# thunlp/OpenMatch

Measured on AMD Instinct MI355X. Metric: passages/sec encode (bert-base DPR bi-encoder, 128 tok -> 768-d) [+ queries/sec exact top-1000 over 8.8M x 768 in `search`], higher is better.
Workload: dtype f16; 1 GPU; bert-base DPR bi-encoder encode+search, MS MARCO 8.8M x 128-tok -> 768-d (BASELINE configs[1]); seq_len=128, global_batch=1024, index_rows=8841823, queries=6980, topk=1000, weights=random-init BertConfig() seed 0, parallelism=shard1

## Files before the change

include/openmatch_hip.h:

```cpp
#ifndef OPENMATCH_HIP_H
#define OPENMATCH_HIP_H

#include <stddef.h>
#include <stdint.h>

#ifdef __cplusplus
extern "C" {
#endif

#define OM_ABI_VERSION 6

#define OM_F32 0
#define OM_BF16 1
#define OM_F16 2

#define OM_ACT_NONE 0
#define OM_ACT_GELU_ERF 1
#define OM_ACT_RELU 2
#define OM_ACT_GELU_TANH 3
#define OM_ACT_SILU 5
#define OM_ACT_MUL_RESID 0x100
#define OM_ACT_PRE_GRAD 0x200

#define OM_ARCH_BERT 0
#define OM_ARCH_T5 1
#define OM_ARCH_MODERNBERT 2

#define OM_ARCH_CAUSAL 3

#define OM_ARCH_NOMICBERT 4

#define OM_POOL_NONE 0
#define OM_POOL_FIRST 1
#define OM_POOL_MEAN 2
#define OM_POOL_LAST 3

#define OM_SEARCH_F32 0
#define OM_SEARCH_F16_RESCORE 1

const char* om_last_error(void);
int om_abi_version(void);

int om_device_count(void);

#define OM_TIMING_GEMM_BF16 0
#define OM_TIMING_GEMM_F32 1
#define OM_TIMING_SCAN 2
void om_debug_gemm_trace(unsigned long long* buf);
void om_debug_gemm_gen(int gen);
#define OM_GEMM_FAMILY_V1 1
#define OM_GEMM_FAMILY_V2 2
#define OM_GEMM_FAMILY_V6 6
#define OM_GEMM_FAMILY_G7 7
#define OM_GEMM_FAMILY_G7_ONE_TILE 70
#define OM_GEMM_FAMILY_G7C16 71
#define OM_GEMM_FAMILY_G7R16 72
#define OM_GEMM_FAMILY_SKINNY 9
int om_debug_gemm_last(void);
int om_debug_gemm_plan(int in_dtype, const void* A, int64_t lda, const void* B, int64_t ldb, int out_dtype, void* C, int64_t ldc,
                       int64_t M, int64_t N, int64_t K, const float* bias, const void* resid, int64_t ldr, int act);
typedef struct OmDebugGemmEpilogue {
  const float* bias; const void* resid; int64_t ldr; int act;
  void* pre_act; int64_t ldp; float drop_p; uint64_t seed; const int* drop_rows;
  const float* ln_stats; const float* ln_colsum; const float* rln_stats; const float* rln_g; const float* rln_b; float* stats_out;
  const void* resid_lo; void* out_lo;
  const float* resid32; float* out32;
  const float* a_ln32; const float* a_ln_g; const float* a_ln_b; float* a_ln_stats_out; const float* rln32; const float* rln32_stats;
  int lo8; float ln_inv_h, ln_eps; int ln_rms; int reverse;
  const int* rows_dev;
} OmDebugGemmEpilogue;
int om_debug_gemm_ex(int in_dtype, const void* A, int64_t lda, const void* B, int64_t ldb, int out_dtype, void* C, int64_t ldc,
                     int64_t M, int64_t N, int64_t K, const OmDebugGemmEpilogue* ep, void* stream);
int om_debug_gemm_plan_ex(int in_dtype, const void* A, int64_t lda, const void* B, int64_t ldb, int out_dtype, void* C, int64_t ldc,
                          int64_t M, int64_t N, int64_t K, const OmDebugGemmEpilogue* ep);
int om_debug_gemm_splitk(int in_dtype, const void* A, int64_t lda, const void* B, int64_t ldb, float* C, int64_t ldc, int64_t M,
                         int64_t N, int64_t K, void* stream);
#define OM_OPT_ENCODER_FUSED_LN 0
#define OM_OPT_ENCODER_DEBUG 1
#define OM_OPT_ATTENTION_FAST 2
#define OM_OPT_SCAN_GEN7 3
#define OM_OPT_SCAN_GROWTH 4
#define OM_OPT_WGRAD_DEBUG 5
#define OM_OPT_GEMM_GROUP_M 6
#define OM_OPT_SCAN_QGROUP 7
#define OM_OPT_TRAIN_WGRAD_STREAM 8
#define OM_OPT_ATTENTION_DEBUG 9
#define OM_OPT_ENCODER_PINGPONG 10
#define OM_OPT_ENCODER_TWO_PLANE 11
#define OM_OPT_GEMM_VARIANT 12
#define OM_OPT_SEARCH_DEBUG 13
#define OM_OPT_TRAIN_WGRAD_BATCH 14
#define OM_OPT_GEMM_MAX_GRID 15
#define OM_OPT_GEMM_CONT 16
#define OM_OPT_TRAIN_TAPE_GRAD 17
#define OM_OPT_TRAIN_RES32 18
#define OM_OPT_GEMM_SKINNY_M 19
#define OM_OPT_GEMM_SKINNY_CFG 20
#define OM_OPT_FEW_ROWS_LN_FUSE 21
#define OM_OPT_ENCODER_SKIP_PAD 22
#define OM_OPT_COUNT 23
int om_debug_option(int opt, int value);
int om_debug_option_value(int opt);
int om_debug_attention(const void* qkv, void* ctx, const int64_t* mask, int64_t B, int L, int H, int heads, void* stream);
int om_debug_attention_ex(int dtype, const void* qkv, void* ctx, const int64_t* mask, const float* pos_bias, int64_t B, int L, int H,
                          int heads, float scale, float drop_p, uint64_t seed, void* stream, int reverse, const int* kmax,
                          const int* cu, int w);
int om_debug_rope(int dtype, void* qkv, int64_t M, int L, int H, float theta, void* stream);
int om_debug_rope_rows(int dtype, void* qkv, int64_t rows, int L, int H, float theta, const int* row_map, void* stream);
int om_debug_swiglu_rows(int dtype, const void* in, void* out, int64_t M, int F, void* stream);
int om_debug_embed(int dtype, const int64_t* ids, const int64_t* type_ids, const float* word, const float* pos, const float* type,
                   const float* g, const float* b, void* out, int64_t M, int L, int H, int vocab, int type_vocab, float eps, void* stream);
int om_debug_attention_causal(int dtype, const void* qkv, void* ctx, const int64_t* mask, int64_t B, int L, int n_heads, int n_kv_heads,
                              float scale, void* stream);
int om_debug_rope_gqa(int dtype, void* qkv, int64_t M, int L, int n_heads, int n_kv_heads, const float* inv_freq, float scaling, void* stream);
int om_debug_attention_causal_packed(int dtype, const void* qkv, void* ctx, const int64_t* mask, const int* cu, int64_t B, int L, int n_heads,
                                     int n_kv_heads, float scale, void* stream);
int om_debug_rope_gqa_rows(int dtype, void* qkv, int64_t rows, int L, int n_heads, int n_kv_heads, const float* inv_freq, float scaling,
                           const int* row_map, void* stream);
int om_debug_attention_causal_hd(int dtype, const void* qkv, void* ctx, const int64_t* mask, int64_t B, int L, int n_heads, int n_kv_heads,
                                 int head_dim, float scale, void* stream);
int om_debug_attention_causal_hd_packed(int dtype, const void* qkv, void* ctx, const int64_t* mask, const int* cu, int64_t B, int L,
                                        int n_heads, int n_kv_heads, int head_dim, float scale, void* stream);
int om_debug_qknorm_rope(int dtype, void* qkv, int64_t M, int L, int n_heads, int n_kv_heads, int head_dim, const float* q_norm_g,
                         const float* k_norm_g, float eps, const float* inv_freq, float scaling, void* stream);
int om_debug_qknorm_rope_rows(int dtype, void* qkv, int64_t rows, int L, int n_heads, int n_kv_heads, int head_dim, const float* q_norm_g,
                              const float* k_norm_g, float eps, const float* inv_freq, float scaling, const int* row_map, void* stream);
int om_debug_attention_gqa_d256(int dtype, const void* qkv, void* ctx, const int64_t* mask, int64_t B, int L, int n_heads, int n_kv_heads,
                                float scale, int w, void* stream);
int om_debug_qknorm_rope_d256(int dtype, void* qkv, int64_t M, int L, int n_heads, int n_kv_heads, const float* q_norm_g, const float* k_norm_g,
                              float eps, const float* inv_freq, float scaling, void* stream);
int om_debug_attention_gqa_d256_packed(int dtype, const void* qkv, void* ctx, const int64_t* mask, const int* cu, int64_t B, int L, int n_heads,
                                       int n_kv_heads, float scale, int w, void* stream);
int om_debug_qknorm_rope_d256_rows(int dtype, void* qkv, int64_t rows, int L, int n_heads, int n_kv_heads, const float* q_norm_g,
                                   const float* k_norm_g, float eps, const float* inv_freq, float scaling, const int* row_map, void* stream);
int om_debug_rmsnorm_add(int dtype, const void* h, int64_t ldh, float* x, int64_t ldx, const float* g, int64_t M, int H, float eps, void* stream);
int om_debug_mask_extent(const int64_t* mask, int64_t B, int L, int* kmax, void* stream);
int om_debug_pack_rows(const int* kmax, int64_t B, int L, int64_t rows, int* cu, int* cls_rows, int* row_map, void* stream);
#define OM_ATTN_FAMILY_GENERIC 1
#define OM_ATTN_FAMILY_FWD16 2
#define OM_ATTN_FAMILY_FWD16_KMAX4 3
#define OM_ATTN_FAMILY_FWD16C 4
#define OM_ATTN_FAMILY_LONG 5
#define OM_ATTN_FAMILY_D32 6
#define OM_ATTN_FAMILY_BAND16 7
#define OM_ATTN_FAMILY_BAND32 8
int om_debug_attention_last(void);
int om_debug_attention_plan(int dtype, int64_t B, int L, int H, int heads, int has_bias, float drop_p, int has_kmax, int has_cu, int w);
#define OM_ATTN_BWD_FAMILY_BWD16 1
#define OM_ATTN_BWD_FAMILY_GENERIC 2
#define OM_ATTN_BWD_FAMILY_LONG 3
#define OM_ATTN_BWD_FAMILY_D32 4
int om_debug_attention_bwd_last(void);
int om_debug_attention_bwd_plan(int dtype, int64_t B, int L, int H, int heads, int has_bias, int has_drel, int has_cu, int packed);
int om_debug_attention_bwd_ex(int dtype, const void* qkv, const void* ctx, const void* dctx, void* dqkv, const int64_t* mask,
                              const float* pos_bias, float* drel, float* stats, int64_t B, int L, int H, int heads, float scale,
                              float drop_p, uint64_t seed, const int* cu, int packed, void* stream);
size_t om_debug_attention_bwd_stats_bytes(int64_t B, int heads);
#define OM_ENC_PATH_BERT_FUSED 1
#define OM_ENC_PATH_BERT_PENDING_LN 2
#define OM_ENC_PATH_BERT_FEW32 3
#define OM_ENC_PATH_BERT_PLAIN 4
#define OM_ENC_PATH_MODERNBERT 5
#define OM_ENC_PATH_T5_FUSED 6
#define OM_ENC_PATH_T5_PLAIN 7
struct OmEncoderConfig;
int om_debug_encoder_plan(const struct OmEncoderConfig* cfg, int gated_ffn, int has_rel_bias, int64_t B, int64_t L, int64_t packed_rows,
                          int want_hidden);
int om_debug_encoder_skip_pad(const struct OmEncoderConfig* cfg, int gated_ffn, int has_rel_bias, int64_t B, int64_t L, int want_hidden);
int om_debug_attn_drop_keep(uint64_t seed, int64_t b, int h, int heads, int Lm, int q, int key, float p);
int om_debug_wave_sum_check(const float* in, float* out_shuffle, float* out_dpp, int64_t groups, void* stream);
#define OM_ROW_FWD_GENERIC 1
#define OM_ROW_FWD_X8 2
#define OM_ROW_LN_BWD 3
int om_debug_row_kernel_last(void);
int om_debug_layernorm(int dtype, const void* x, int64_t ldx, void* y, int64_t ldy, const float* g, const float* b, int64_t M, int H,
                       float eps, int rms, const void* x_lo, int lo8, void* stream);
int om_debug_layernorm_f32out(int dtype, const void* x, int64_t ldx, float* y, int64_t ldy, const float* g, const float* b, int64_t M,
                              int H, float eps, int rms, const void* x_lo, const int* rows, int lo8, void* stream);
int om_debug_layernorm_from_f32(int dtype, const float* x, int64_t ldx, void* y, int64_t ldy, const float* g, const float* b, int64_t M,
                                int H, float eps, int rms, void* stream);
int om_debug_layernorm_dual(int dtype, const float* x, int64_t ldx, void* y, float* y32, int64_t ldy, const float* g, const float* b,
                            int64_t M, int H, float eps, void* stream);
int om_debug_norm_bwd(int dtype, const void* dy, const void* x, const float* g, void* dx, float* dg, float* db, int64_t M, int H,
                      float eps, int rms, const void* add, void* stream);
int om_debug_ln_bwd_drop(int dtype, const void* dy, const void* x, const float* g, void* dx, void* dx_drop, float drop_p,
                         uint64_t drop_seed, float* dg, float* db, int64_t M, int H, float eps, const float* dy32, const float* x32,
                         float* partial, int* partial_blocks , const int* drop_rows, void* stream);
typedef struct OmLnSite { const float* partial; float* dg; float* db; int blocks; } OmLnSite;
int om_debug_ln_param_reduce(const OmLnSite* sites , int n, int H, void* stream);
int om_debug_embed_bwd(int dtype, const void* dy, const int64_t* ids, const int64_t* type_ids, const float* word, const float* pos,
                       const float* type, const float* g, float* dword, float* dpos, float* dtype_, float* dg, float* db, int64_t M,
                       int L, int H, int vocab, int type_vocab, float eps, const int* cu, void* stream);
int om_debug_pool(int dtype, const void* x, const int64_t* mask, float* out, int64_t B, int L, int H, int mode, const int* cu,
                  void* stream);
int om_debug_pool_bwd(int dtype, const float* dp, const int64_t* mask, void* dh, int64_t B, int L, int H, int mode, const int* cu,
                      void* stream);
int om_debug_l2norm(const float* x, float* y, int64_t M, int D, void* stream);
int om_debug_l2norm_bwd(const float* x, const float* dy, float* dx, int64_t M, int D, void* stream);
int om_debug_colsum(int dtype, const void* x, int64_t ld, int64_t M, int N, float* out, void* stream);
int om_debug_dropout(int dtype, const void* x, void* y, int64_t n, float p, uint64_t seed, const int* rows, int H, void* stream);
int om_debug_ln_fold(int dtype, const void* W, const float* gamma, const float* beta, const float* b, void* Wf, float* colsum,
                     float* bf, int N, int K, void* stream);
int om_debug_ln_stats_reduce(const float* slots, int nslots, int64_t M, float* out, void* stream);
int om_kernel_timing_enable(int enable);
int om_kernel_timing_read(int kernel_class, double* total_ms, int64_t* launches, double* flops);

int om_gemm_nt(int in_dtype, const void* A, int64_t lda, const void* B, int64_t ldb,
               int out_dtype, void* C, int64_t ldc, int64_t M, int64_t N, int64_t K,
               const float* bias, const void* resid, int64_t ldr, int act, void* stream);

int om_gemm_tn_acc(int in_dtype, const void* A, int64_t lda, const void* B, int64_t ldb,
                   float* C, int64_t ldc, float* bias, int64_t M, int64_t N, int64_t K, void* stream);

typedef struct OmTnProblem {
  const void* A; const void* B; float* C; float* bias;
  int64_t lda, ldb, ldc, N, K;
} OmTnProblem;
int om_gemm_tn_acc_batch(int in_dtype, const OmTnProblem* problems, int n, int64_t M, void* stream);

typedef struct OmLayerWeights {
  const void* qkv_w;
  const float* qkv_b;
  const void* o_w;
  const float* o_b;
  const float* ln1_g;
  const float* ln1_b;
  const void* ffn1_w;
  const float* ffn1_b;
  const void* ffn1g_w;
  const void* ffn2_w;
  const float* ffn2_b;
  const float* ln2_g;
  const float* ln2_b;
} OmLayerWeights;

typedef struct OmEncoderConfig {
  int arch;
  int dtype;
  int hidden;
  int n_layers;
  int n_heads;
  int head_dim;
  int ffn;
  int vocab;
  int max_pos;
  int type_vocab;
  int act;
  float ln_eps;
  int rel_buckets;
  int rel_max_dist;
  int pooling;
  int head_in;
  int head_out;
  int normalize;
  float rope_theta_global;
  float rope_theta_local;
  int half_window;
  uint64_t sliding_layers;
} OmEncoderConfig;

typedef struct OmEncoderWeights {
  const float* word_emb;
  const float* pos_emb;
  const float* type_emb;
  const float* emb_ln_g;
  const float* emb_ln_b;
  const OmLayerWeights* layers_host;
  const float* final_ln_g;
  const float* rel_bias;
  const float* head_w;
  const void* folded;
  const float* final_ln_b;
} OmEncoderWeights;

size_t om_encoder_fold_bytes(const OmEncoderConfig* cfg);
int om_encoder_fold_weights(const OmEncoderConfig* cfg, const OmEncoderWeights* w, void* folded, size_t bytes, void* stream);

size_t om_encoder_workspace_bytes(const OmEncoderConfig* cfg, int64_t B, int64_t L);

int om_t5_relative_bucket(int relative_position, int num_buckets, int max_distance);

int om_encoder_forward(const OmEncoderConfig* cfg, const OmEncoderWeights* w,
                       const int64_t* input_ids, const int64_t* attention_mask,
                       const int64_t* token_type_ids, int64_t B, int64_t L,
                       void* out_hidden, float* out_reps, void* workspace,
                       size_t workspace_bytes, void* stream);

int om_encoder_packed_supported(const OmEncoderConfig* cfg, int gated_ffn, int64_t B, int64_t L, int64_t packed_rows);
size_t om_encoder_workspace_bytes_packed(const OmEncoderConfig* cfg, int64_t B, int64_t L, int64_t packed_rows);
int om_encoder_forward_packed(const OmEncoderConfig* cfg, const OmEncoderWeights* w,
                              const int64_t* input_ids, const int64_t* attention_mask,
                              const int64_t* token_type_ids, int64_t B, int64_t L, int64_t packed_rows,
                              float* out_reps, void* workspace, size_t workspace_bytes, void* stream);

typedef struct OmCausalConfig {
  OmEncoderConfig base;
  int n_kv_heads;
  float rope_attention_scaling;
  float inv_freq[32];
} OmCausalConfig;
size_t om_causal_encoder_workspace_bytes(const OmCausalConfig* cfg, int64_t B, int64_t L);
int om_causal_encoder_forward(const OmCausalConfig* cfg, const OmEncoderWeights* w, const int64_t* input_ids,
                              const int64_t* attention_mask, int64_t B, int64_t L, void* out_hidden, float* out_reps,
                              void* workspace, size_t workspace_bytes, void* stream);
int om_causal_encoder_packed_supported(const OmCausalConfig* cfg, int64_t B, int64_t L, int64_t packed_rows);
size_t om_causal_encoder_workspace_bytes_packed(const OmCausalConfig* cfg, int64_t B, int64_t L, int64_t packed_rows);
int om_causal_encoder_forward_packed(const OmCausalConfig* cfg, const OmEncoderWeights* w, const int64_t* input_ids,
                                     const int64_t* attention_mask, int64_t B, int64_t L, int64_t packed_rows, float* out_reps,
                                     void* workspace, size_t workspace_bytes, void* stream);

typedef struct OmCausalConfig2 {
  OmCausalConfig base;
  int qk_norm;
  int reserved;
  float inv_freq[64];
} OmCausalConfig2;
typedef struct OmCausalQkNorm {
  const float* q_norm_g;
  const float* k_norm_g;
} OmCausalQkNorm;
size_t om_causal2_encoder_workspace_bytes(const OmCausalConfig2* cfg, int64_t B, int64_t L);
// ... 204 lines not shown
```

openmatch_amd/csrc/abi.cpp:

```cpp
#include "common.h"

static thread_local std::string g_last_error;
void om_set_error(const std::string& msg) { g_last_error = msg; }

extern "C" const char* om_last_error(void) { return g_last_error.c_str(); }
extern "C" int om_abi_version(void) { return OM_ABI_VERSION; }
extern "C" int om_device_count(void) {
  int n = 0;
  hipError_t e = hipGetDeviceCount(&n);
  if (e != hipSuccess) {
    om_set_error(std::string("hipGetDeviceCount: ") + hipGetErrorString(e));
    return -1;
  }
  return n;
}

#include <mutex>
#include <vector>
namespace {
struct Span { hipEvent_t a, b; };
struct ClassStat { std::vector<Span> spans; double flops = 0; size_t used = 0; };
bool g_timing = false;
ClassStat g_stat[3];
std::mutex g_mu;
}
bool om_timing_on() { return g_timing; }
void om_timing_begin(int c, hipStream_t s) {
  std::lock_guard<std::mutex> lk(g_mu);
  ClassStat& st = g_stat[c];
  if (st.used == st.spans.size()) {
    Span sp;
    (void)hipEventCreate(&sp.a);
    (void)hipEventCreate(&sp.b);
    st.spans.push_back(sp);
  }
  (void)hipEventRecord(st.spans[st.used].a, s);
}
void om_timing_end(int c, hipStream_t s, double flops) {
  std::lock_guard<std::mutex> lk(g_mu);
  ClassStat& st = g_stat[c];
  (void)hipEventRecord(st.spans[st.used].b, s);
  st.used++;
  st.flops += flops;
}
extern "C" int om_kernel_timing_enable(int enable) { g_timing = enable != 0; return 0; }
extern "C" int om_kernel_timing_read(int c, double* total_ms, int64_t* launches, double* flops) {
  if (c < 0 || c > 2) { om_set_error("om_kernel_timing_read: bad class"); return 1; }
  std::lock_guard<std::mutex> lk(g_mu);
  ClassStat& st = g_stat[c];
  double ms = 0;
  for (size_t i = 0; i < st.used; ++i) {
    hipError_t e = hipEventSynchronize(st.spans[i].b);
    float t = 0;
    if (e == hipSuccess) e = hipEventElapsedTime(&t, st.spans[i].a, st.spans[i].b);
    if (e != hipSuccess) { om_set_error(std::string("om_kernel_timing_read: ") + hipGetErrorString(e)); return 1; }
    ms += t;
  }
  if (total_ms) *total_ms = ms;
  if (launches) *launches = (int64_t)st.used;
  if (flops) *flops = st.flops;
  st.used = 0; st.flops = 0;
  return 0;
}

#include <atomic>
#include <map>
#include <tuple>
namespace {
std::atomic<int> g_opt[OM_OPT_COUNT];
std::atomic<bool> g_opt_init{false};
std::mutex g_opt_mu;
void opt_init() {
  std::lock_guard<std::mutex> lk(g_opt_mu);
  if (g_opt_init.load()) return;
  const char* e = getenv("OM_ENCODER_FUSED_LN");
  g_opt[OM_OPT_ENCODER_FUSED_LN] = e ? atoi(e) : 1;
  g_opt[OM_OPT_ENCODER_DEBUG] = getenv("OM_ENCODER_DEBUG") ? 1 : 0;
  e = getenv("OM_ATTENTION_FAST");
  g_opt[OM_OPT_ATTENTION_FAST] = e ? atoi(e) : 1;
  e = getenv("OM_SCAN_GEN7");
  g_opt[OM_OPT_SCAN_GEN7] = e ? atoi(e) : 1;
  e = getenv("OM_SCAN_GROWTH");
  g_opt[OM_OPT_SCAN_GROWTH] = e ? atoi(e) : 60;
  g_opt[OM_OPT_WGRAD_DEBUG] = 0;
  g_opt[OM_OPT_ATTENTION_DEBUG] = 0;
  e = getenv("OM_ENCODER_PINGPONG");
  g_opt[OM_OPT_ENCODER_PINGPONG] = e ? atoi(e) : 1;
  e = getenv("OM_TRAIN_WGRAD_STREAM");
  g_opt[OM_OPT_TRAIN_WGRAD_STREAM] = e ? atoi(e) : 1;
  e = getenv("OM_SCAN_QGROUP");
  g_opt[OM_OPT_SCAN_QGROUP] = e ? atoi(e) : 8;
  e = getenv("OM_GEMM_GROUP_M");
  g_opt[OM_OPT_GEMM_GROUP_M] = e ? atoi(e) : 8;
  e = getenv("OM_ENCODER_TWO_PLANE");
  g_opt[OM_OPT_ENCODER_TWO_PLANE] = e ? atoi(e) : 3;
  e = getenv("OM_GEMM_VARIANT");
  g_opt[OM_OPT_GEMM_VARIANT] = e ? atoi(e) : 0;
  e = getenv("OM_SEARCH_DEBUG");
  g_opt[OM_OPT_SEARCH_DEBUG] = e ? (atoi(e) ? atoi(e) : 1) : 0;
  e = getenv("OM_TRAIN_WGRAD_BATCH");
  g_opt[OM_OPT_TRAIN_WGRAD_BATCH] = e ? atoi(e) : 4;
  e = getenv("OM_GEMM_MAX_GRID");
  g_opt[OM_OPT_GEMM_MAX_GRID] = e ? atoi(e) : 0;
  e = getenv("OM_TRAIN_TAPE_GRAD");
  g_opt[OM_OPT_TRAIN_TAPE_GRAD] = e ? atoi(e) : 1;
  e = getenv("OM_TRAIN_RES32");
  g_opt[OM_OPT_TRAIN_RES32] = e ? atoi(e) : 1;
  e = getenv("OM_GEMM_CONT");
  g_opt[OM_OPT_GEMM_CONT] = e ? atoi(e) : 495;
  e = getenv("OM_GEMM_SKINNY_M");
  g_opt[OM_OPT_GEMM_SKINNY_M] = e ? atoi(e) : 1024;
  e = getenv("OM_FEW_ROWS_LN_FUSE");
  g_opt[OM_OPT_FEW_ROWS_LN_FUSE] = e ? atoi(e) : 64;
  e = getenv("OM_ENCODER_SKIP_PAD");
  g_opt[OM_OPT_ENCODER_SKIP_PAD] = e ? atoi(e) : 1;
  g_opt_init.store(true);
}
}
bool om_option_is_set(int opt) {
  if (opt == OM_OPT_SCAN_GROWTH) return getenv("OM_SCAN_GROWTH") != nullptr;
  return false;
}
int om_option(int opt) {
  if (!g_opt_init.load(std::memory_order_acquire)) opt_init();
  return g_opt[opt].load(std::memory_order_relaxed);
}
extern "C" int om_debug_option(int opt, int value) {
  if (opt < 0 || opt >= OM_OPT_COUNT) { om_set_error("om_debug_option: unknown option"); return 1; }
  if (!g_opt_init.load(std::memory_order_acquire)) opt_init();
  g_opt[opt].store(value);
  return 0;
}
extern "C" int om_debug_option_value(int opt) {
  if (opt < 0 || opt >= OM_OPT_COUNT) { om_set_error("om_debug_option_value: unknown option"); return -1; }
  return om_option(opt);
}

int om_t5_lut_device(int L, int buckets, int max_dist, const int** out) {
  static std::mutex mu;
  static std::map<std::tuple<int, int, int, int>, int*> cache;
  int dev = 0;
  OM_HIP(hipGetDevice(&dev));
  std::lock_guard<std::mutex> lk(mu);
  auto key = std::make_tuple(dev, L, buckets, max_dist);
  auto it = cache.find(key);
  if (it == cache.end()) {
    std::vector<int> lut(2 * L);
    for (int rel = -(L - 1); rel <= L - 1; ++rel) lut[rel + (L - 1)] = om_t5_relative_bucket(rel, buckets, max_dist);
    int* d = nullptr;
    OM_HIP(hipMalloc(&d, (size_t)(2 * L) * sizeof(int)));
    OM_HIP(hipMemcpy(d, lut.data(), (size_t)(2 * L - 1) * sizeof(int), hipMemcpyHostToDevice));
    it = cache.emplace(key, d).first;
  }
  *out = it->second;
  return 0;
}
```

openmatch_amd/csrc/attention.hip:

```cpp
#include <type_traits>

#include "attn_chunked.h"
#include "attn_plan.h"

static thread_local int g_attn_last = 0;
extern "C" int om_debug_attention_last(void) { return g_attn_last; }

template <typename T, int KT>
__global__ __launch_bounds__(64 * KT) void attention_kernel(
    const T* __restrict__ qkv, T* __restrict__ ctx, const int64_t* __restrict__ mask,
    const float* __restrict__ pos_bias, int L, int H, int heads, float scale, float drop_p,
    uint64_t seed) {
  typedef AttnGeom<T> G;
  typedef typename MmaOps<T>::frag_t frag_t;
  constexpr int LP = KT * 32 + 4;
  extern __shared__ __attribute__((aligned(16))) char smem[];
  char* sK = smem;
  T* sVt = (T*)(smem + KT * 32 * G::ROWB);
  float* sM = (float*)(smem + KT * 32 * G::ROWB + 64 * LP * (int)sizeof(T));

  const int h = blockIdx.x % heads;
  const int64_t b = blockIdx.x / heads;
  const int tid = threadIdx.x, nthr = blockDim.x;
  const int64_t ld = 3 * (int64_t)H;
// ... 262 lines not shown
    }
  char* const out = (char*)(ctx + (row0 + q0) * (int64_t)H + h * 64);
#pragma unroll
  for (int it = 0; it < 4; ++it) {
    const int row = it * 8 + (lane >> 3), c = lane & 7;
    const uint4 v = *(const uint4*)(so + row * 128 + ((c ^ (row & 7)) << 4));
    if (!(DBG & 4) || v.x == 0x12345u) { if (q0 + row < L) *(uint4*)(out + (int64_t)row * H * 2 + c * 16) = v; }
  }
}

template <typename T, int KT, bool BIAS, bool DROP, int DBG = 0>
__global__ __launch_bounds__(64 * KT, KT <= 4 ? ((BIAS || DROP) ? 3 : 4) : 2) void attention_fwd16_kernel(
    const T* __restrict__ qkv, T* __restrict__ ctx, const int64_t* __restrict__ mask,
    const float* __restrict__ pos_bias, int L, int H, int heads, float scale, float drop_p, uint64_t seed, int rev,
    const int* __restrict__ kmax, const int* __restrict__ cu) {
#define OM_ATTN_BODY(V) attention_fwd16_body<T, KT, BIAS, DROP, DBG, V>(qkv, ctx, mask, pos_bias, Lb, H, heads, scale, drop_p, seed, rev, row0, L)
  const int64_t b = rev ? (int64_t)(gridDim.x / heads) - 1 - blockIdx.x / heads : blockIdx.x / heads;
  int64_t row0 = b * L;
  int Lb = L;
  if (cu) {
    const int c0 = __builtin_amdgcn_readfirstlane(cu[b]), c1 = __builtin_amdgcn_readfirstlane(cu[b + 1]);
    row0 = c0; Lb = c1 - c0;
    if (Lb <= 0) return;
  }
  if (KT == 4 && !BIAS && !DROP && (kmax || cu)) {
    const int kt = ((cu ? Lb : __builtin_amdgcn_readfirstlane(kmax[b])) + 31) >> 5;
    if (kt <= 1) { OM_ATTN_BODY(1); return; }
    if (kt == 2) { OM_ATTN_BODY(2); return; }
    if (kt == 3) { OM_ATTN_BODY(3); return; }
  }
  OM_ATTN_BODY(KT);
#undef OM_ATTN_BODY
}

template <typename T, int KT, bool BIAS, bool DROP>
static int launch_attn16(const void* qkv, void* ctx, const int64_t* mask, const float* pos_bias, int64_t B, int L, int H,
                         int heads, float scale, float drop_p, uint64_t seed, hipStream_t s, int rev, const int* kmax, const int* cu) {
  const int lds = 2 * KT * 32 * 128 + KT * 32 * 4;
  if (attn_lds_once<attention_fwd16_kernel<T, KT, BIAS, DROP>>(lds)) return 1;
#ifdef OM_PROBE_KERNELS
  const int dbg = (sizeof(T) == 2 && std::is_same<T, bf16_t>::value && KT == 4 && !BIAS && !DROP) ? om_option(OM_OPT_ATTENTION_DEBUG) : 0;
#else
  const int dbg = 0;
#endif
  if (dbg) {
#ifdef OM_PROBE_KERNELS
#define OM_ATTN_DBG(D)                                                                                                        \
  case D:                                                                                                                     \
    hipLaunchKernelGGL((attention_fwd16_kernel<bf16_t, 4, false, false, D>), dim3((unsigned)(heads * B)), dim3(256), lds, s,          \
                       (const bf16_t*)qkv, (bf16_t*)ctx, mask, pos_bias, L, H, heads, scale, drop_p, seed, rev, kmax, cu);    \
    break;
    switch (dbg) { OM_ATTN_DBG(1) OM_ATTN_DBG(2) OM_ATTN_DBG(3) OM_ATTN_DBG(4) OM_ATTN_DBG(5) OM_ATTN_DBG(6) OM_ATTN_DBG(7) default: break; }
#undef OM_ATTN_DBG
#endif
    OM_LAUNCH_CHECK();
    return 0;
  }
  hipLaunchKernelGGL((attention_fwd16_kernel<T, KT, BIAS, DROP>), dim3((unsigned)(heads * B)), dim3(64 * KT), lds, s, (const T*)qkv,
                     (T*)ctx, mask, pos_bias, L, H, heads, scale, drop_p, seed, rev, kmax, cu);
  OM_LAUNCH_CHECK();
  return 0;
}
template <typename T, bool BIAS, bool DROP>
__global__ __launch_bounds__(256, 2) void attention_fwd16c_kernel(
    const T* __restrict__ qkv, T* __restrict__ ctx, const int64_t* __restrict__ mask,
    const float* __restrict__ pos_bias, int Lm, int H, int heads, float scale, float drop_p, uint64_t seed, const int* __restrict__ cu) {
  const int h = blockIdx.x % heads;
  const int64_t b = blockIdx.x / heads;
  int64_t row0 = b * Lm;
  int L = Lm;
  if (cu) {
    const int c0 = __builtin_amdgcn_readfirstlane(cu[b]), c1 = __builtin_amdgcn_readfirstlane(cu[b + 1]);
    row0 = c0; L = c1 - c0;
  }
  const int qb = blockIdx.y * 128;
  if (qb >= L) return;
  attn_chunked16<T, AttnFull, BIAS, DROP>(attn_rows_fused(qkv, ctx, row0, H, h), AttnFull{}, mask + b * Lm, L, L, qb, scale, AttnFullArgs{pos_bias, drop_p, seed, b, h, heads, Lm});
}

template <typename T, bool BIAS, bool DROP>
static int launch_attn16c(const void* qkv, void* ctx, const int64_t* mask, const float* pos_bias, int64_t B, int L, int H,
                           int heads, float scale, float drop_p, uint64_t seed, hipStream_t s, const int* cu) {
  const int lds = 2 * 128 * 128 + 128 * 4;
  hipLaunchKernelGGL((attention_fwd16c_kernel<T, BIAS, DROP>), dim3((unsigned)(heads * B), (unsigned)((L + 127) / 128)), dim3(256), lds, s,
                     (const T*)qkv, (T*)ctx, mask, pos_bias, L, H, heads, scale, drop_p, seed, cu);
  OM_LAUNCH_CHECK();
  return 0;
}
template <typename T>
__global__ __launch_bounds__(256) void attention_long_kernel(
    const T* __restrict__ qkv, T* __restrict__ ctx, const int64_t* __restrict__ mask,
    const float* __restrict__ pos_bias, int Lm, int H, int heads, float scale, float drop_p, uint64_t seed, const int* __restrict__ cu) {
  const int h = blockIdx.x % heads;
  const int64_t b = blockIdx.x / heads;
  const int qb = blockIdx.y * 128;
  int64_t row0 = b * Lm;
  int L = Lm;
  if (cu) { row0 = cu[b]; L = cu[b + 1] - cu[b]; }
  if (qb >= L) return;
  attn_chunked_qreg<T, AttnFull>(attn_rows_fused(qkv, ctx, row0, H, h), AttnFull{}, mask + b * Lm, L, L, qb, scale, AttnFullArgs{pos_bias, drop_p, seed, b, h, heads, Lm});
}

template <typename T>
static int launch_attn_long(const void* qkv, void* ctx, const int64_t* mask, const float* pos_bias, int64_t B, int L, int H,
                            int heads, float scale, float drop_p, uint64_t seed, hipStream_t s, const int* cu) {
  const int lds = 128 * AttnGeom<T>::ROWB + 64 * 132 * (int)sizeof(T) + 128 * 4 + 128 * 4;
  if (attn_lds_once<attention_long_kernel<T>>(lds)) return 1;
  hipLaunchKernelGGL((attention_long_kernel<T>), dim3((unsigned)(heads * B), (unsigned)((L + 127) / 128)), dim3(256), lds, s,
                     (const T*)qkv, (T*)ctx, mask, pos_bias, L, H, heads, scale, drop_p, seed, cu);
  OM_LAUNCH_CHECK();
  return 0;
}

template <typename T, int KT>
static int launch_attn(const void* qkv, void* ctx, const int64_t* mask, const float* pos_bias,
                       int64_t B, int L, int H, int heads, float scale, float drop_p, uint64_t seed,
                       hipStream_t s) {
  constexpr int LP = KT * 32 + 4;
  const int lds = KT * 32 * AttnGeom<T>::ROWB + 64 * LP * (int)sizeof(T) + KT * 32 * 4;
  if (attn_lds_once<attention_kernel<T, KT>>(lds)) return 1;
  const int waves = (L + 31) / 32;
  hipLaunchKernelGGL((attention_kernel<T, KT>), dim3((unsigned)(heads * B)),
                     dim3(64 * waves), lds, s, (const T*)qkv, (T*)ctx, mask, pos_bias, L, H, heads,
                     scale, drop_p, seed);
  OM_LAUNCH_CHECK();
  return 0;
}

__global__ void mask_extent_kernel(const int64_t* __restrict__ mask, int64_t B, int L, int* __restrict__ kmax) {
  const int64_t b = (int64_t)blockIdx.x * (blockDim.x >> 6) + (threadIdx.x >> 6);
  if (b >= B) return;
  const int lane = threadIdx.x & 63;
  int last = 0;
  for (int k = lane; k < L; k += 64) if (mask[b * L + k] != 0) last = k + 1;
#pragma unroll
  for (int o = 32; o > 0; o >>= 1) last = max(last, __shfl_xor(last, o, 64));
  if (lane == 0) kmax[b] = last ? last : L;
}
__global__ __launch_bounds__(1024) void pack_rows_kernel(const int* __restrict__ kmax, int64_t B, int L, int64_t rows, int* __restrict__ cu,
                                                          int* __restrict__ cls_rows, int* __restrict__ row_map) {
  __shared__ int part[1024];
  const int tid = threadIdx.x;
  const int64_t per = (B + 1023) / 1024, lo = tid * per, hi = lo + per < B ? lo + per : B;
  int sum = 0;
  for (int64_t i = lo; i < hi; ++i) sum += kmax[i];
  part[tid] = sum;
  __syncthreads();
  for (int off = 1; off < 1024; off <<= 1) {
    const int v = tid >= off ? part[tid - off] : 0;
    __syncthreads();
    part[tid] += v;
    __syncthreads();
  }
  int run = part[tid] - sum;
  const int cap = (int)rows;
  for (int64_t i = lo; i < hi; ++i) {
    cu[i] = run < cap ? run : cap;
    cls_rows[i] = run < cap ? run : cap - 1;
    const int n = kmax[i];
    for (int k = 0; k < n; ++k) if (run + k < cap) row_map[run + k] = (int)(i * L + k);
    run += n;
  }
  const int total = part[1023];
  if (tid == 1023) { cu[B] = total < cap ? total : cap; cu[B + 1] = total; }
  for (int64_t t = total + tid; t < rows; t += 1024) row_map[t] = -1;
}
int omk_pack_rows(const int* kmax, int64_t B, int L, int64_t rows, int* cu, int* cls_rows, int* row_map, hipStream_t s) {
  if (B <= 0) return 0;
  if (rows > 0x7fffffff || B * (int64_t)L > 0x7fffffff) OM_FAIL("packed rows: token counts below 2^31");
  hipLaunchKernelGGL(pack_rows_kernel, dim3(1), dim3(1024), 0, s, kmax, B, L, rows, cu, cls_rows, row_map);
  OM_LAUNCH_CHECK();
  return 0;
}

int omk_mask_extent(const int64_t* mask, int64_t B, int L, int* kmax, hipStream_t s) {
  if (B <= 0) return 0;
  hipLaunchKernelGGL(mask_extent_kernel, dim3((unsigned)((B + 3) / 4)), dim3(256), 0, s, mask, B, L, kmax);
  OM_LAUNCH_CHECK();
  return 0;
}

int omk_attention(int dtype, const void* qkv, void* ctx, const int64_t* mask, const float* pos_bias, int64_t B, int L, int H, int heads,
                  float scale, float drop_p, uint64_t seed, hipStream_t s, int reverse, const int* kmax, const int* cu, int w) {
  g_attn_last = 0;
  const AttnPlan p = attn_plan_fwd(dtype, B, L, H, heads, pos_bias != nullptr, drop_p, kmax != nullptr, cu != nullptr, w, attn_switches());
  if (p.error) OM_FAIL(p.error);
  g_attn_last = p.family | (p.kt << 8);
  switch (p.family) {
    case 0: return 0;
    case OM_ATTN_FAMILY_D32: return omk_attention_d32(p, dtype, qkv, ctx, mask, pos_bias, B, L, H, heads, scale, drop_p, seed, s, reverse, kmax, cu);
    case OM_ATTN_FAMILY_BAND16: case OM_ATTN_FAMILY_BAND32: return omk_attention_band(dtype, qkv, ctx, mask, B, L, H, heads, scale, w, kmax, s);
    case OM_ATTN_FAMILY_FWD16: case OM_ATTN_FAMILY_FWD16_KMAX4:
      return attn_with_type16(dtype, [&](auto t) {
        return attn_with_kt<1, 2, 4, 6, 8>(p.kt, [&](auto kt) {
          return attn_with_flags(p.bias, p.drop, [&](auto bias, auto drop) {
            return launch_attn16<decltype(t), kt(), bias(), drop()>(qkv, ctx, mask, pos_bias, B, L, H, heads, scale, drop_p, seed, s, reverse, kmax, cu);
          });
        });
      });
    case OM_ATTN_FAMILY_FWD16C:
      return attn_with_type16(dtype, [&](auto t) {
        return attn_with_flags(p.bias, p.drop, [&](auto bias, auto drop) {
          return launch_attn16c<decltype(t), bias(), drop()>(qkv, ctx, mask, pos_bias, B, L, H, heads, scale, drop_p, seed, s, cu);
        });
      });
    case OM_ATTN_FAMILY_LONG:
      return attn_with_type(dtype, [&](auto t) { return launch_attn_long<decltype(t)>(qkv, ctx, mask, pos_bias, B, L, H, heads, scale, drop_p, seed, s, cu); });
    default:
      if (dtype == OM_BF16)
        return attn_with_kt<1, 2, 4, 6, 8>(p.kt, [&](auto kt) { return launch_attn<bf16_t, kt()>(qkv, ctx, mask, pos_bias, B, L, H, heads, scale, drop_p, seed, s); });
      return attn_with_kt<1, 2, 4, 6, 8>(p.kt, [&](auto kt) { return launch_attn<float, kt()>(qkv, ctx, mask, pos_bias, B, L, H, heads, scale, drop_p, seed, s); });
  }
}

extern "C" int om_debug_attention_plan(int dtype, int64_t B, int L, int H, int heads, int has_bias, float drop_p, int has_kmax, int has_cu, int w) {
  const AttnPlan p = attn_plan_fwd(dtype, B, L, H, heads, has_bias != 0, drop_p, has_kmax != 0, has_cu != 0, w, attn_switches());
  if (p.error) { om_set_error(std::string(__func__) + ": " + p.error); return -1; }
  return p.family | (p.kt << 8);
}

extern "C" int om_debug_attention_ex(int dtype, const void* qkv, void* ctx, const int64_t* mask, const float* pos_bias, int64_t B, int L, int H,
                                     int heads, float scale, float drop_p, uint64_t seed, void* stream, int reverse, const int* kmax,
                                     const int* cu, int w) {
  g_attn_last = 0;
  if (!qkv || !ctx || !mask) OM_FAIL("null argument");
  if (dtype != OM_F32 && dtype != OM_BF16 && dtype != OM_F16) OM_FAIL("attention: dtype must be OM_F32, OM_BF16 or OM_F16");
  if (w > 0 && (pos_bias || drop_p > 0.f || cu || reverse)) OM_FAIL("banded attention: no position bias, dropout, packed rows or reverse walk");
  return omk_attention(dtype, qkv, ctx, mask, pos_bias, B, L, H, heads, scale, drop_p, seed, (hipStream_t)stream, reverse, kmax, cu, w);
}
extern "C" int om_debug_attention(const void* qkv, void* ctx, const int64_t* mask, int64_t B, int L, int H, int heads, void* stream) {
  return om_debug_attention_ex(OM_BF16, qkv, ctx, mask, nullptr, B, L, H, heads, 0.125f, 0.f, 0, stream, 0, nullptr, nullptr, 0);
}
extern "C" int om_debug_rope(int dtype, void* qkv, int64_t M, int L, int H, float theta, void* stream) {
  if (!qkv) OM_FAIL("null argument");
  if (dtype != OM_F32 && dtype != OM_BF16 && dtype != OM_F16) OM_FAIL("rotary positions: dtype must be OM_F32, OM_BF16 or OM_F16");
  return omk_rope(dtype, qkv, M, L, H, theta, (hipStream_t)stream);
}
extern "C" int om_debug_rope_rows(int dtype, void* qkv, int64_t rows, int L, int H, float theta, const int* row_map, void* stream) {
  if (!qkv || !row_map) OM_FAIL("null argument");
  if (dtype != OM_F32 && dtype != OM_BF16 && dtype != OM_F16) OM_FAIL("rotary positions: dtype must be OM_F32, OM_BF16 or OM_F16");
  return omk_rope(dtype, qkv, rows, L, H, theta, (hipStream_t)stream, row_map);
}
extern "C" int om_debug_mask_extent(const int64_t* mask, int64_t B, int L, int* kmax, void* stream) {
  if (!mask || !kmax) OM_FAIL("null argument");
  if (L < 1) OM_FAIL("mask extent: L must be at least 1");
  return omk_mask_extent(mask, B, L, kmax, (hipStream_t)stream);
}
extern "C" int om_debug_pack_rows(const int* kmax, int64_t B, int L, int64_t rows, int* cu, int* cls_rows, int* row_map, void* stream) {
  if (!kmax || !cu || !cls_rows || !row_map) OM_FAIL("null argument");
  if (rows < 1) OM_FAIL("packed rows: rows must be at least 1");
  return omk_pack_rows(kmax, B, L, rows, cu, cls_rows, row_map, (hipStream_t)stream);
}
extern "C" int om_debug_attn_drop_keep(uint64_t seed, int64_t b, int h, int heads, int Lm, int q, int key, float p) {
  return attn_drop_keep1(seed, b, h, heads, Lm, q, key, AttnDrop(p).thresh) ? 1 : 0;
}
```

openmatch_amd/csrc/elementwise.hip:

```cpp
#include "common.h"
#include "kernels.h"
#include "ln_row.h"
#include <type_traits>

#define ROWS_PER_BLOCK 4
#define MAX_VEC_LIMIT 8

template <typename TOut, int MAX_VEC>
__device__ inline void norm_and_store(float (&x)[MAX_VEC][4], int nvec, int lane, int H,
                                      const float* __restrict__ g, const float* __restrict__ b,
                                      float eps, int rms, TOut* __restrict__ out, float* __restrict__ out32 = nullptr) {
  float mean, rstd;
  ln_row_stats<MAX_VEC>(x, nvec, lane, H, eps, rms, mean, rstd);
#pragma unroll
  for (int j = 0; j < MAX_VEC; ++j) {
    const int c = (lane + 64 * j) * 4;
    if (j < nvec && c < H) {
      float gv[4], y[4];
      Vec4<float>::load(g + c, gv);
      if (b) {
        float bv[4];
        Vec4<float>::load(b + c, bv);
#pragma unroll
        for (int e = 0; e < 4; ++e) y[e] = ln_affine(x[j][e], mean, rstd, gv[e], bv[e]);
// ... 178 lines not shown
  float v[MAX_VEC][4];
  if (bert) {
    int64_t tt = type_ids ? type_ids[row] : 0;
    tt = tt < 0 ? 0 : (tt >= type_vocab ? type_vocab - 1 : tt);
    const int t = (int)(row % L);
#pragma unroll
    for (int j = 0; j < MAX_VEC; ++j) {
      const int c = (lane + 64 * j) * 4;
      if (j < nvec && c < H) {
        float w[4], ty[4], p[4];
        Vec4<float>::load(word + id * H + c, w);
        if (type && pos) {
          Vec4<float>::load(type + tt * H + c, ty);
          Vec4<float>::load(pos + (int64_t)t * H + c, p);
#pragma unroll
          for (int e = 0; e < 4; ++e) v[j][e] = (w[e] + ty[e]) + p[e];
        } else if (type) {
          Vec4<float>::load(type + tt * H + c, ty);
#pragma unroll
          for (int e = 0; e < 4; ++e) v[j][e] = w[e] + ty[e];
        } else if (pos) {
          Vec4<float>::load(pos + (int64_t)t * H + c, p);
#pragma unroll
          for (int e = 0; e < 4; ++e) v[j][e] = w[e] + p[e];
        } else {
#pragma unroll
          for (int e = 0; e < 4; ++e) v[j][e] = w[e];
        }
      }
    }
    norm_and_store<TOut, MAX_VEC>(v, nvec, lane, H, g, b, eps, 0, out + orow * H, out32 ? out32 + orow * H : nullptr);
  } else {
#pragma unroll
    for (int j = 0; j < MAX_VEC; ++j) {
      const int c = (lane + 64 * j) * 4;
      if (j < nvec && c < H) {
        Vec4<float>::load(word + id * H + c, v[j]);
        Vec4<TOut>::store(out + orow * H + c, v[j]);
      }
    }
  }
}

template <typename T>
__global__ void pool_kernel(const T* __restrict__ x, const int64_t* __restrict__ mask,
                            float* __restrict__ out, int L, int H, int mode, const int* __restrict__ cu) {
  const int64_t b = blockIdx.x;
  const T* xb = x + (cu ? (int64_t)cu[b] : b * (int64_t)L) * H;
  const int Lb = cu ? cu[b + 1] - cu[b] : L;
  for (int c = threadIdx.x * 4; c < H; c += blockDim.x * 4) {
    float acc[4] = {0.f, 0.f, 0.f, 0.f};
    if (mode == OM_POOL_FIRST) {
      Vec4<T>::load(xb + c, acc);
    } else {
      float cnt = 0.f;
      for (int t = 0; t < Lb; ++t) {
        const float m = (float)mask[b * L + t];
        float v[4];
        Vec4<T>::load(xb + (int64_t)t * H + c, v);
#pragma unroll
        for (int e = 0; e < 4; ++e) acc[e] += v[e] * m;
        cnt += m;
      }
      cnt = fmaxf(cnt, 1e-9f);
#pragma unroll
      for (int e = 0; e < 4; ++e) acc[e] = acc[e] / cnt;
    }
    Vec4<float>::store(out + b * H + c, acc);
  }
}

__global__ __launch_bounds__(64 * ROWS_PER_BLOCK) void l2norm_kernel(const float* __restrict__ x,
                                                                     float* __restrict__ y,
                                                                     int64_t M, int D) {
  const int lane = threadIdx.x & 63;
  const int64_t row = (int64_t)blockIdx.x * ROWS_PER_BLOCK + (threadIdx.x >> 6);
  if (row >= M) return;
  float ss = 0.f;
  for (int c = lane; c < D; c += 64) { const float v = x[row * D + c]; ss += v * v; }
  const float denom = fmaxf(sqrtf(wave_sum(ss)), 1e-12f);
  for (int c = lane; c < D; c += 64) y[row * D + c] = x[row * D + c] / denom;
}

__global__ void t5_bias_kernel(const float* __restrict__ table, const int* __restrict__ lut,
                               float* __restrict__ out, int L, int heads) {
  const int64_t n = (int64_t)heads * L * L;
  for (int64_t i = (int64_t)blockIdx.x * blockDim.x + threadIdx.x; i < n;
       i += (int64_t)gridDim.x * blockDim.x) {
    const int k = (int)(i % L), q = (int)((i / L) % L), h = (int)(i / ((int64_t)L * L));
    out[i] = table[lut[k - q + (L - 1)] * heads + h];
  }
}

__global__ __launch_bounds__(64 * ROWS_PER_BLOCK) void index_to_f16_kernel(
    const float* __restrict__ x, f16_t* __restrict__ y, int64_t N, int d,
    unsigned* stats) {
  const int lane = threadIdx.x & 63;
  const int64_t row = (int64_t)blockIdx.x * ROWS_PER_BLOCK + (threadIdx.x >> 6);
  if (row >= N) return;
  float e2 = 0.f, n2 = 0.f;
  for (int c = lane; c < d; c += 64) {
    const float v = x[row * d + c];
    const f16_t r = (f16_t)v;
    const float rv = (float)r;
    y[row * d + c] = r;
    e2 += (v - rv) * (v - rv);
    n2 += rv * rv;
  }
  e2 = wave_sum(e2); n2 = wave_sum(n2);
  if (lane == 0) {
    const unsigned ue = __float_as_uint(sqrtf(e2) * 1.0001f), un = __float_as_uint(sqrtf(n2) * 1.0001f);
    if (ue > stats[0]) atomicMax(stats + 0, ue);
    if (un > stats[1]) atomicMax(stats + 1, un);
  }
}

static thread_local int g_row_last = 0;
void omk_row_note(int word) { g_row_last = word; }
extern "C" int om_debug_row_kernel_last(void) { return g_row_last; }
template <typename T> constexpr int row_dt() { return sizeof(T) == 4 ? OM_F32 : (std::is_same<T, bf16_t>::value ? OM_BF16 : OM_F16); }
static inline int row_fwd_word(int body, int nv, int tin, int tout, bool plane, bool lo8) {
  return body | nv << 4 | tin << 8 | tout << 12 | (plane ? 1 << 16 : 0) | (plane && lo8 ? 1 << 17 : 0);
}

template <typename TIn, typename TOut>
static int launch_ln(const void* x, int64_t ldx, void* y, int64_t ldy, const float* g,
                     const float* b, int64_t M, int H, float eps, int rms, hipStream_t s, const int* rows = nullptr) {
  const unsigned grid = (unsigned)((M + ROWS_PER_BLOCK - 1) / ROWS_PER_BLOCK);
  omk_row_note(row_fwd_word(OM_ROW_FWD_GENERIC, H <= 1024 ? 4 : 8, row_dt<TIn>(), row_dt<TOut>(), false, false));
  if (H <= 1024)
    hipLaunchKernelGGL((layernorm_kernel<TIn, TOut, 4>), dim3(grid), dim3(64 * ROWS_PER_BLOCK), 0, s,
                       (const TIn*)x, ldx, (TOut*)y, ldy, g, b, M, H, eps, rms, rows);
  else
    hipLaunchKernelGGL((layernorm_kernel<TIn, TOut, 8>), dim3(grid), dim3(64 * ROWS_PER_BLOCK), 0, s,
                       (const TIn*)x, ldx, (TOut*)y, ldy, g, b, M, H, eps, rms, rows);
  OM_LAUNCH_CHECK();
  return 0;
}

__global__ __launch_bounds__(256) void ln_stats_reduce_kernel(const float2* __restrict__ slots, int nslots, int64_t M, float2* __restrict__ out) {
  const int64_t m = (int64_t)blockIdx.x * 256 + threadIdx.x;
  if (m >= M) return;
  float s1 = 0.f, s2 = 0.f;
  for (int k = 0; k < nslots; ++k) { const float2 v = slots[(int64_t)k * M + m]; s1 += v.x; s2 += v.y; }
  out[m] = make_float2(s1, s2);
}
int omk_ln_stats_reduce(const float* slots, int nslots, int64_t M, float* out, hipStream_t s) {
  if (M <= 0) return 0;
  hipLaunchKernelGGL(ln_stats_reduce_kernel, dim3((unsigned)((M + 255) / 256)), dim3(256), 0, s, (const float2*)slots, nslots, M, (float2*)out);
  OM_LAUNCH_CHECK();
  return 0;
}

int omk_layernorm_from_f32(int dtype, const float* x, int64_t ldx, void* y, int64_t ldy, const float* g, const float* b, int64_t M, int H,
                           float eps, int rms, hipStream_t s) {
  if (H % 4 != 0 || H > 64 * 4 * MAX_VEC_LIMIT) OM_FAIL("hidden size must be a multiple of 4 and <= 2048");
  if (M <= 0) return 0;
  if (dtype == OM_BF16) return launch_ln<float, bf16_t>(x, ldx, y, ldy, g, b, M, H, eps, rms, s);
  if (dtype == OM_F16) return launch_ln<float, f16_t>(x, ldx, y, ldy, g, b, M, H, eps, rms, s);
  return launch_ln<float, float>(x, ldx, y, ldy, g, b, M, H, eps, rms, s);
}

template <typename TIn, int MAX_VEC>
__global__ __launch_bounds__(64 * ROWS_PER_BLOCK) void rmsnorm_add_kernel(const TIn* __restrict__ h, int64_t ldh, float* __restrict__ x, int64_t ldx,
                                                                          const float* __restrict__ g, int64_t M, int H, float eps) {
  const int lane = threadIdx.x & 63;
  const int64_t row = (int64_t)blockIdx.x * ROWS_PER_BLOCK + (threadIdx.x >> 6);
  if (row >= M) return;
  const int nvec = (H / 4 + 63) / 64;
  float v[MAX_VEC][4];
#pragma unroll
  for (int j = 0; j < MAX_VEC; ++j) {
    const int c = (lane + 64 * j) * 4;
    if (j < nvec && c < H) Vec4<TIn>::load(h + row * ldh + c, v[j]);
  }
  float mean, rstd;
  ln_row_stats<MAX_VEC>(v, nvec, lane, H, eps, 1, mean, rstd);
  float* const xr = x + row * ldx;
#pragma unroll
  for (int j = 0; j < MAX_VEC; ++j) {
    const int c = (lane + 64 * j) * 4;
    if (j < nvec && c < H) {
      float gv[4], xv[4];
      Vec4<float>::load(g + c, gv);
      Vec4<float>::load(xr + c, xv);
#pragma unroll
      for (int e = 0; e < 4; ++e) xv[e] = __fadd_rn(xv[e], __fmul_rn(__fmul_rn(v[j][e], rstd), gv[e]));
      Vec4<float>::store(xr + c, xv);
    }
  }
}

template <typename TIn>
static void launch_rmsnorm_add(const void* h, int64_t ldh, float* x, int64_t ldx, const float* g, int64_t M, int H, float eps, hipStream_t s) {
  const unsigned grid = (unsigned)((M + ROWS_PER_BLOCK - 1) / ROWS_PER_BLOCK);
  if (H <= 1024) hipLaunchKernelGGL((rmsnorm_add_kernel<TIn, 4>), dim3(grid), dim3(64 * ROWS_PER_BLOCK), 0, s, (const TIn*)h, ldh, x, ldx, g, M, H, eps);
  else hipLaunchKernelGGL((rmsnorm_add_kernel<TIn, 8>), dim3(grid), dim3(64 * ROWS_PER_BLOCK), 0, s, (const TIn*)h, ldh, x, ldx, g, M, H, eps);
}

int omk_rmsnorm_add(int dtype, const void* h, int64_t ldh, float* x, int64_t ldx, const float* g, int64_t M, int H, float eps, hipStream_t s) {
  if (H % 4 != 0 || H > 64 * 4 * MAX_VEC_LIMIT) OM_FAIL("hidden size must be a multiple of 4 and <= 2048");
  if (ldh % 4 || ldx % 4) OM_FAIL("norm-add: row pitches of whole four-element vectors");
  if (M <= 0) return 0;
  if (dtype == OM_BF16) launch_rmsnorm_add<bf16_t>(h, ldh, x, ldx, g, M, H, eps, s);
  else if (dtype == OM_F16) launch_rmsnorm_add<f16_t>(h, ldh, x, ldx, g, M, H, eps, s);
  else launch_rmsnorm_add<float>(h, ldh, x, ldx, g, M, H, eps, s);
  OM_LAUNCH_CHECK();
  return 0;
}

int omk_layernorm_f32out(int dtype, const void* x, int64_t ldx, float* y, int64_t ldy, const float* g, const float* b,
                         int64_t M, int H, float eps, int rms, hipStream_t s, const void* x_lo, const int* rows, int lo8) {
  if (lo8 && !(x_lo && dtype == OM_F16 && H % 256 == 0 && ldx % H == 0)) OM_FAIL("eight-bit second plane: float16 rows of a whole-tile [M, H] tensor");
  if (H % 4 != 0 || H > 64 * 4 * MAX_VEC_LIMIT) OM_FAIL("hidden size must be a multiple of 4 and <= 2048");
  if (M <= 0) return 0;
  if ((dtype == OM_BF16 || (dtype == OM_F16 && x_lo)) && H % 8 == 0 && H <= 1024 && ldx % 8 == 0 && ldy % 4 == 0 &&
      !(((uintptr_t)x | (uintptr_t)y | (uintptr_t)x_lo) & 15) && !(((uintptr_t)g | (uintptr_t)b) & 15)) {
    const unsigned grid = (unsigned)((M + 7) / 8);
    const int nv = (H / 8 + 31) / 32;
#define LN8F_(NV, TI) hipLaunchKernelGGL((layernorm_bf16x8_kernel<NV, float, TI>), dim3(grid), dim3(256), 0, s, (const TI*)x, ldx, \
                                    y, ldy, g, b, M, H, eps, rms, (const TI*)x_lo, rows, lo8)
#define LN8F(NV) do { if (dtype == OM_BF16) LN8F_(NV, bf16_t); else LN8F_(NV, f16_t); } while (0)
    omk_row_note(row_fwd_word(OM_ROW_FWD_X8, nv <= 1 ? 1 : nv, dtype, OM_F32, x_lo != nullptr, lo8 != 0));
    if (nv <= 1) LN8F(1); else if (nv == 2) LN8F(2); else if (nv == 3) LN8F(3); else LN8F(4);
#undef LN8F
#undef LN8F_
    OM_LAUNCH_CHECK();
    return 0;
  }
  if (x_lo) OM_FAIL("two-plane LayerNorm input: 16-bit rows of whole 16-byte vectors only");
  if (dtype == OM_BF16) return launch_ln<bf16_t, float>(x, ldx, y, ldy, g, b, M, H, eps, rms, s, rows);
  if (dtype == OM_F16) return launch_ln<f16_t, float>(x, ldx, y, ldy, g, b, M, H, eps, rms, s, rows);
  return launch_ln<float, float>(x, ldx, y, ldy, g, b, M, H, eps, rms, s, rows);
}

__global__ void pack_overflow_poison_kernel(const int* __restrict__ cu, int64_t B, int64_t rows, float* __restrict__ out, int64_t n) {
  if ((int64_t)cu[B + 1] <= rows) return;
  for (int64_t i = (int64_t)blockIdx.x * blockDim.x + threadIdx.x; i < n; i += (int64_t)gridDim.x * blockDim.x) out[i] = __int_as_float(0x7fc00000);
}
int omk_pack_overflow_poison(const int* cu, int64_t B, int64_t rows, float* out, int64_t n, hipStream_t s) {
  if (n <= 0) return 0;
  hipLaunchKernelGGL(pack_overflow_poison_kernel, dim3(64), dim3(256), 0, s, cu, B, rows, out, n);
  OM_LAUNCH_CHECK();
  return 0;
}

int omk_layernorm_dual(int dtype, const float* x, int64_t ldx, void* y, float* y32, int64_t ldy, const float* g, const float* b,
                       int64_t M, int H, float eps, hipStream_t s) {
  if (H % 4 != 0 || H > 64 * 4 * MAX_VEC_LIMIT) OM_FAIL("hidden size must be a multiple of 4 and <= 2048");
  if (M <= 0) return 0;
  const unsigned grid = (unsigned)((M + ROWS_PER_BLOCK - 1) / ROWS_PER_BLOCK);
#define LND(TO, MV) hipLaunchKernelGGL((layernorm_kernel<float, TO, MV>), dim3(grid), dim3(64 * ROWS_PER_BLOCK), 0, s, x, ldx, (TO*)y, ldy, g, b, M, \
                                       H, eps, 0, (const int*)nullptr, y32)
  if (dtype != OM_BF16 && dtype != OM_F16) OM_FAIL("a 16-bit output format");
  omk_row_note(row_fwd_word(OM_ROW_FWD_GENERIC, H <= 1024 ? 4 : 8, OM_F32, dtype, false, false));
  if (dtype == OM_BF16) { if (H <= 1024) LND(bf16_t, 4); else LND(bf16_t, 8); }
  else { if (H <= 1024) LND(f16_t, 4); else LND(f16_t, 8); }
#undef LND
  OM_LAUNCH_CHECK();
  return 0;
}

int omk_layernorm(int dtype, const void* x, int64_t ldx, void* y, int64_t ldy, const float* g,
                  const float* b, int64_t M, int H, float eps, int rms, hipStream_t s, const void* x_lo, int lo8) {
  if (lo8 && !(x_lo && dtype == OM_F16 && H % 256 == 0 && ldx % H == 0)) OM_FAIL("eight-bit second plane: float16 rows of a whole-tile [M, H] tensor");
  if (H % 4 != 0 || H > 64 * 4 * MAX_VEC_LIMIT) OM_FAIL("hidden size must be a multiple of 4 and <= 2048");
  if (M <= 0) return 0;
  if (x_lo && !((dtype == OM_BF16 || dtype == OM_F16) && H % 8 == 0 && H <= 1024 && ldx % 8 == 0 && ldy % 8 == 0 &&
                !(((uintptr_t)x | (uintptr_t)y | (uintptr_t)x_lo) & 15) && !(((uintptr_t)g | (uintptr_t)b) & 15)))
    OM_FAIL("two-plane LayerNorm input: 16-bit rows of whole 16-byte vectors only");
  if ((dtype == OM_BF16 || (dtype == OM_F16 && x_lo)) && H % 8 == 0 && H <= 1024 && ldx % 8 == 0 && ldy % 8 == 0 &&
      !(((uintptr_t)x | (uintptr_t)y) & 15) && !(((uintptr_t)g | (uintptr_t)b) & 15)) {
    const unsigned grid = (unsigned)((M + 7) / 8);
    const int nv = (H / 8 + 31) / 32;
#define LN8_(NV, TI) hipLaunchKernelGGL((layernorm_bf16x8_kernel<NV, TI, TI>), dim3(grid), dim3(256), 0, s, (const TI*)x, ldx, \
                                   (TI*)y, ldy, g, b, M, H, eps, rms, (const TI*)x_lo, (const int*)nullptr, lo8)
#define LN8(NV) do { if (dtype == OM_BF16) LN8_(NV, bf16_t); else LN8_(NV, f16_t); } while (0)
    omk_row_note(row_fwd_word(OM_ROW_FWD_X8, nv <= 1 ? 1 : nv, dtype, dtype, x_lo != nullptr, lo8 != 0));
    if (nv <= 1) LN8(1); else if (nv == 2) LN8(2); else if (nv == 3) LN8(3); else LN8(4);
#undef LN8
#undef LN8_
    OM_LAUNCH_CHECK();
    return 0;
  }
  if (dtype == OM_BF16) return launch_ln<bf16_t, bf16_t>(x, ldx, y, ldy, g, b, M, H, eps, rms, s);
  if (dtype == OM_F16) return launch_ln<f16_t, f16_t>(x, ldx, y, ldy, g, b, M, H, eps, rms, s);
  return launch_ln<float, float>(x, ldx, y, ldy, g, b, M, H, eps, rms, s);
}

int omk_embed(int dtype, const int64_t* ids, const int64_t* type_ids, const float* word,
              const float* pos, const float* type, const float* g, const float* b, void* out,
              int64_t M, int L, int H, int vocab, int type_vocab, float eps, int bert,
              hipStream_t s, const int* row_map, float* out32) {
  if (H % 4 != 0 || H > 64 * 4 * MAX_VEC_LIMIT) OM_FAIL("hidden size must be a multiple of 4 and <= 2048");
  if (M <= 0) return 0;
  if (out32 && (!bert || row_map)) OM_FAIL("embedding: the f32 copy goes with the BERT LayerNorm on unpacked rows");
  const unsigned grid = (unsigned)((M + ROWS_PER_BLOCK - 1) / ROWS_PER_BLOCK);
#define EMBED_LAUNCH(TT, NV)                                                                   \
  hipLaunchKernelGGL((embed_kernel<TT, NV>), dim3(grid), dim3(64 * ROWS_PER_BLOCK), 0, s, ids, \
                     type_ids, word, pos, type, g, b, (TT*)out, M, L, H, vocab, type_vocab, eps, bert, row_map, out32)
  if (dtype == OM_BF16) {
    if (H <= 1024) EMBED_LAUNCH(bf16_t, 4); else EMBED_LAUNCH(bf16_t, 8);
  } else if (dtype == OM_F16) {
    if (H <= 1024) EMBED_LAUNCH(f16_t, 4); else EMBED_LAUNCH(f16_t, 8);
  } else {
    if (H <= 1024) EMBED_LAUNCH(float, 4); else EMBED_LAUNCH(float, 8);
// ... 171 lines not shown
```

openmatch_amd/csrc/encoder.hip:

```cpp
#include <math.h>

#include <stdlib.h>

#include <algorithm>
#include <map>
#include <mutex>
#include <utility>
#include <vector>

#include "encoder_plan.h"

namespace {
struct FoldSlot { size_t w, cs, bf; };
struct FoldLayout { size_t per_layer, total; FoldSlot qkv, ffn1; };
FoldLayout fold_layout(const OmEncoderConfig* c) {
  const size_t H = c->hidden, F = enc_ffn1_cols(c);
  size_t off = 0;
  auto take = [&](size_t bytes) { size_t o = off; off = align_up(off + bytes, 256); return o; };
  FoldLayout L;
  L.qkv.w = take(3 * H * H * 2); L.qkv.cs = take(3 * H * 4); L.qkv.bf = take(3 * H * 4);
  L.ffn1.w = take(F * H * 2); L.ffn1.cs = take(F * 4); L.ffn1.bf = take(F * 4);
  L.per_layer = off;
  L.total = off * (size_t)c->n_layers;
  return L;
// ... 3 lines not shown
}
}

extern "C" size_t om_encoder_fold_bytes(const OmEncoderConfig* cfg) {
  if (!cfg || !fold_applies(cfg)) return 0;
  return fold_layout(cfg).total;
}

extern "C" int om_encoder_fold_weights(const OmEncoderConfig* c, const OmEncoderWeights* w, void* blob, size_t bytes, void* stream) {
  if (!c || !w || !blob) OM_FAIL("null argument");
  if (!fold_applies(c)) OM_FAIL("nothing to fold for this configuration (om_encoder_fold_bytes is 0)");
  const FoldLayout L = fold_layout(c);
  if (bytes < L.total || ((uintptr_t)blob & 255)) OM_FAIL("fold buffer too small or not 256-byte aligned");
  const OmLayerWeights* Ls = w->layers_host;
  if (!Ls) OM_FAIL("layers_host is null");
  hipStream_t s = (hipStream_t)stream;
  const int H = c->hidden, F = enc_ffn1_cols(c);
  const bool bert = enc_bert_family(c);
  for (int l = 0; l < c->n_layers; ++l) {
    char* base = (char*)blob + (size_t)l * L.per_layer;
    const OmLayerWeights& lw = Ls[l];
    if (l > 0) {
      const float* g = bert ? Ls[l - 1].ln2_g : lw.ln1_g;
      const float* beta = bert ? Ls[l - 1].ln2_b : nullptr;
      if (omk_ln_fold(c->dtype, lw.qkv_w, g, beta, bert ? lw.qkv_b : nullptr, base + L.qkv.w, (float*)(base + L.qkv.cs),
                      (float*)(base + L.qkv.bf), 3 * H, H, s)) return 1;
    }
    if (!lw.ffn1g_w) {
      const float* g = bert ? lw.ln1_g : lw.ln2_g;
      const float* beta = bert ? lw.ln1_b : nullptr;
      if (omk_ln_fold(c->dtype, lw.ffn1_w, g, beta, bert ? lw.ffn1_b : nullptr, base + L.ffn1.w, (float*)(base + L.ffn1.cs),
                      (float*)(base + L.ffn1.bf), F, H, s)) return 1;
    }
  }
  return 0;
}

static int folded_weights(const OmEncoderConfig* c, const OmEncoderWeights* w, int layer, bool ffn1, const void* W, const float* g,
                          const float* beta, const float* b, int N, int K, void* scratch_w, float* scratch_cs, float* scratch_bf,
                          hipStream_t s, const void** Wf, const float** cs, const float** bf) {
  if (w->folded) {
    const FoldLayout L = fold_layout(c);
    const char* base = (const char*)w->folded + (size_t)layer * L.per_layer;
    const FoldSlot& sl = ffn1 ? L.ffn1 : L.qkv;
    *Wf = base + sl.w; *cs = (const float*)(base + sl.cs); *bf = (const float*)(base + sl.bf);
    return 0;
  }
  if (omk_ln_fold(c->dtype, W, g, beta, b, scratch_w, scratch_cs, scratch_bf, N, K, s)) return 1;
  *Wf = scratch_w; *cs = scratch_cs; *bf = scratch_bf;
  return 0;
}

struct EncWs {
  char *x, *y, *x1, *qkv, *ctx, *ff, *ff2;
  float *pooled, *headout, *posbias;
  float* final32;
  int* lut;
  int* kmax;
  int *cu, *cls_rows, *row_map;
  char* wfold;
  float *colsum, *bfold, *stats1, *stats2, *slots;
  char *y_lo, *x1_lo;
  float *r32a, *r32b, *y32;
  size_t total;
};

static EncWs carve(const OmEncoderConfig* c, const EncPlan& p, int64_t B, int64_t L, int64_t packed_rows, char* base) {
  const bool half = c->dtype == OM_BF16 || c->dtype == OM_F16;
  const size_t es = half ? 2 : 4;
  const size_t Mreal = (size_t)p.M, M = (size_t)p.Mp, H = c->hidden, F = c->ffn, F1 = enc_ffn1_cols(c);
  const bool bertf = enc_bert_family(c);
  size_t off = 0;
  auto take = [&](size_t bytes) { size_t o = off; off = align_up(off + bytes, 256); return base + o; };
  EncWs w;
  w.x = take(M * H * es);
  w.y = take(M * H * es);
  w.x1 = take(M * H * es);
  w.qkv = take(M * 3 * H * es);
  w.ctx = take(M * H * es);
  w.ff = take(M * F1 * es);
  w.ff2 = take(c->arch == OM_ARCH_T5 || c->arch == OM_ARCH_MODERNBERT || c->arch == OM_ARCH_NOMICBERT ? M * F * es : 0);
  w.pooled = (float*)take((size_t)B * H * 4);
  w.headout = (float*)take((size_t)B * (c->head_out > 0 ? c->head_out : 1) * 4);
  const bool rel = c->arch == OM_ARCH_T5 || (c->arch == OM_ARCH_BERT && c->rel_buckets > 0);
  w.posbias = (float*)take(rel ? (size_t)c->n_heads * L * L * 4 : 0);
  w.lut = (int*)take(rel ? (size_t)(2 * L) * 4 : 0);
  w.kmax = (int*)take((size_t)B * 4);
  w.cu = (int*)take(packed_rows > 0 ? (size_t)(B + 2) * 4 : 0);
  w.cls_rows = (int*)take(packed_rows > 0 ? (size_t)B * 4 : 0);
  w.row_map = (int*)take(packed_rows > 0 ? (size_t)packed_rows * 4 : 0);
  w.final32 = (float*)take(half && c->pooling != OM_POOL_NONE ? (c->pooling == OM_POOL_FIRST ? (size_t)B : Mreal) * H * 4 : 0);
  const bool fuse = half && c->arch != OM_ARCH_MODERNBERT;
  const size_t wide = std::max((size_t)3 * H, F1);
  w.wfold = take(fuse ? wide * H * es : 0);
  w.colsum = (float*)take(fuse ? wide * 4 : 0);
  w.bfold = (float*)take(fuse ? wide * 4 : 0);
  w.stats1 = (float*)take(fuse ? (size_t)2 * c->n_layers * M * 8 : 0);
  w.stats2 = w.stats1 ? w.stats1 + (size_t)c->n_layers * M * 2 : nullptr;
  w.slots = (float*)take(fuse ? (size_t)2 * ((H + 255) / 256) * M * 8 : 0);
  const bool two = fuse && bertf;
  w.y_lo = take(two ? M * H * es : 0);
  w.x1_lo = take(two ? M * H * es : 0);
  w.r32a = (float*)take(p.alloc_few32 ? Mreal * H * 4 : 0);
  w.r32b = (float*)take(p.alloc_few32 ? Mreal * H * 4 : 0);
  w.y32 = (float*)take(p.alloc_few32 ? Mreal * H * 4 : 0);
  w.total = off;
  return w;
}

static size_t workspace_bytes(const OmEncoderConfig* c, int64_t B, int64_t L, int64_t packed_rows) {
  const EncPlan p = encoder_plan_checked(EncPlanIn{c, B, L, packed_rows, false, false, false, false}, encoder_switches());
  return carve(c, p, B, L, packed_rows, nullptr).total;
}

extern "C" size_t om_encoder_workspace_bytes(const OmEncoderConfig* cfg, int64_t B, int64_t L) {
  if (!cfg || B <= 0 || L <= 0) return 0;
  return workspace_bytes(cfg, B, L, 0);
}

extern "C" size_t om_encoder_workspace_bytes_packed(const OmEncoderConfig* cfg, int64_t B, int64_t L, int64_t packed_rows) {
  if (!cfg || B <= 0 || L <= 0 || packed_rows <= 0) return 0;
  return workspace_bytes(cfg, B, L, packed_rows);
}

extern "C" int om_encoder_packed_supported(const OmEncoderConfig* c, int gated_ffn, int64_t B, int64_t L, int64_t packed_rows) {
  return encoder_packed_ok(c, gated_ffn != 0, B, L, packed_rows, encoder_switches()) ? 1 : 0;
}

extern "C" int om_debug_encoder_plan(const OmEncoderConfig* c, int gated_ffn, int has_rel_bias, int64_t B, int64_t L, int64_t packed_rows,
                                     int want_hidden) {
  if (!c) {
    om_set_error("om_debug_encoder_plan: null argument");
    return -1;
  }
  const EncPlan p = encoder_plan(EncPlanIn{c, B, L, packed_rows, want_hidden != 0, gated_ffn != 0, has_rel_bias != 0, c->type_vocab > 0},
                                 encoder_switches());
  if (p.error) {
    om_set_error(std::string("om_debug_encoder_plan: ") + p.error);
    return -1;
  }
  return p.path | (int)p.few_rows << 8 | (int)p.two << 9 | p.lo8 << 10;
}

extern "C" int om_debug_encoder_skip_pad(const OmEncoderConfig* c, int gated_ffn, int has_rel_bias, int64_t B, int64_t L, int want_hidden) {
  if (!c) {
    om_set_error("om_debug_encoder_skip_pad: null argument");
    return -1;
  }
  const EncPlanIn in = {c, B, L, 0, want_hidden != 0, gated_ffn != 0, has_rel_bias != 0, c->type_vocab > 0};
  const EncSwitches sw = encoder_switches();
  return encoder_skip_pad(in, encoder_plan(in, sw), sw) ? 1 : 0;
}

extern "C" int om_t5_relative_bucket(int relative_position, int num_buckets, int max_distance) {
  int nb = num_buckets / 2;
  int bucket = relative_position > 0 ? nb : 0;
  const int n = relative_position < 0 ? -relative_position : relative_position;
  const int max_exact = nb / 2;
  if (n < max_exact) return bucket + n;
  const double v = log((double)n / max_exact) / log((double)max_distance / max_exact) * (nb - max_exact);
  int large = max_exact + (int)v;
  if (large > nb - 1) large = nb - 1;
  return bucket + large;
}

static int check_cfg(const OmEncoderConfig* c) {
  if (const char* why = encoder_cfg_error(c)) OM_FAIL(why);
  return 0;
}

struct EncCall {
  const OmEncoderConfig* c;
  const OmEncoderWeights* w;
  const int64_t* mask;
  int64_t B, L;
  const EncPlan& p;
  const EncWs& ws;
  const float* posbias;
  const int* cu;
  const int* row_map;
  void* out_hidden;
  hipStream_t s;
  const int* rows_dev;
};

struct EncStream {
  const void* x;
  const void* x_lo;
  int lo8;
  const float *g, *b;
  int rms;
  void* spare;
  char* hidden;
  const float* rows32;
};

#define GEMM(A_, lda_, W_, ldw_, C_, ldc_, N_, K_, bias_, res_, ldr_, act_)                        \
  do {                                                                                             \
    if (om_gemm_nt(dt, A_, lda_, W_, ldw_, dt, C_, ldc_, Mg, N_, K_, bias_, res_, ldr_, act_, s)) \
      return 1;                                                                                    \
  } while (0)
#define RUN(expr) do { if (expr) return 1; } while (0)
#define ENC_LOCALS                                                                                                   \
  const OmEncoderConfig* c = k.c; const EncWs& ws = k.ws; const OmLayerWeights* Ls = k.w->layers_host; hipStream_t s = k.s;     \
  const int dt = c->dtype, H = c->hidden, F = c->ffn, nh = c->n_heads;                                              \
  const int64_t B = k.B, L = k.L, M = k.p.M, Mg = k.p.Mg
#define NOMIC_LOCALS                                                                                                 \
  const bool nomic = c->arch == OM_ARCH_NOMICBERT;                                                                   \
  const int F1 = enc_ffn1_cols(c), act1 = nomic ? OM_ACT_NONE : c->act;                                             \
  const void* const ffa = nomic ? ws.ff2 : ws.ff
#define NOMIC_ROPE() do { if (nomic) RUN(omk_rope(dt, ws.qkv, M, (int)L, H, c->rope_theta_global, s, k.row_map)); } while (0)
#define NOMIC_SWIGLU() do { if (nomic) RUN(omk_swiglu_rows(dt, ws.ff, ws.ff2, Mg, F, s)); } while (0)

static int bert_fused(const EncCall& k, EncStream* out) {
  ENC_LOCALS;
  NOMIC_LOCALS;
  const float scale = 1.0f / sqrtf((float)c->head_dim);
  const float inv_h = 1.0f / (float)H;
  const bool two = k.p.two;
  const int lo8 = k.p.lo8;
  const int nslots = 2 * (H / 256);
  const bool pingpong = k.p.pingpong;
  int walk = 1;
#define OM_WALK() (pingpong ? (walk ^= 1, walk ^ 1) : 0)
  for (int l = 0; l < c->n_layers; ++l) {
    const OmLayerWeights& lw = Ls[l];
    float* st1 = ws.stats1 + (size_t)l * Mg * 2;
    float* st2 = ws.stats2 + (size_t)l * Mg * 2;
    const float* st2p = l ? ws.stats2 + (size_t)(l - 1) * Mg * 2 : nullptr;
    GemmEpilogue e = {};
    if (l == 0) {
      e.bias = lw.qkv_b; e.reverse = OM_WALK(); e.rows_dev = k.rows_dev;
      RUN(omk_gemm(dt, ws.x, H, lw.qkv_w, H, dt, ws.qkv, 3 * H, Mg, 3 * H, H, e, s));
    } else {
      const OmLayerWeights& pw = Ls[l - 1];
      const void* wf; const float *cs, *bfp;
      RUN(folded_weights(c, k.w, l, false, lw.qkv_w, pw.ln2_g, pw.ln2_b, lw.qkv_b, 3 * H, H, ws.wfold, ws.colsum, ws.bfold, s, &wf, &cs, &bfp));
      e.bias = bfp; e.ln_stats = st2p; e.ln_colsum = cs; e.ln_inv_h = inv_h; e.ln_eps = c->ln_eps; e.reverse = OM_WALK(); e.rows_dev = k.rows_dev;
      RUN(omk_gemm(dt, ws.x1, H, wf, H, dt, ws.qkv, 3 * H, Mg, 3 * H, H, e, s));
    }
    NOMIC_ROPE();
    RUN(omk_attention(dt, ws.qkv, ws.ctx, k.mask, k.posbias, B, (int)L, H, nh, scale, 0.f, 0, s, OM_WALK(), ws.kmax, k.cu));
    e = GemmEpilogue{};
    e.bias = lw.o_b; e.ldr = H; e.stats_out = ws.slots; e.ln_inv_h = inv_h; e.ln_eps = c->ln_eps;
    if (two) { e.out_lo = ws.y_lo; e.lo8 = lo8; }
    if (l == 0) {
      e.resid = ws.x;
    } else {
      const OmLayerWeights& pw = Ls[l - 1];
      e.resid = ws.x1; e.rln_stats = st2p; e.rln_g = pw.ln2_g; e.rln_b = pw.ln2_b;
      if (two) e.resid_lo = ws.x1_lo;
    }
    e.reverse = OM_WALK(); e.rows_dev = k.rows_dev;
    RUN(omk_gemm(dt, ws.ctx, H, lw.o_w, H, dt, ws.y, H, Mg, H, H, e, s));
    RUN(omk_ln_stats_reduce(ws.slots, nslots, Mg, st1, s));
    const void* wf1; const float *cs1, *bf1;
    RUN(folded_weights(c, k.w, l, true, lw.ffn1_w, lw.ln1_g, lw.ln1_b, lw.ffn1_b, F1, H, ws.wfold, ws.colsum, ws.bfold, s, &wf1, &cs1, &bf1));
    e = GemmEpilogue{};
    e.bias = bf1; e.act = act1; e.ln_stats = st1; e.ln_colsum = cs1; e.ln_inv_h = inv_h; e.ln_eps = c->ln_eps;
    e.reverse = OM_WALK(); e.rows_dev = k.rows_dev;
    RUN(omk_gemm(dt, ws.y, H, wf1, H, dt, ws.ff, F1, Mg, F1, H, e, s));
    NOMIC_SWIGLU();
    e = GemmEpilogue{};
    e.bias = lw.ffn2_b; e.resid = ws.y; e.ldr = H; e.rln_stats = st1; e.rln_g = lw.ln1_g; e.rln_b = lw.ln1_b;
    e.stats_out = ws.slots; e.ln_inv_h = inv_h; e.ln_eps = c->ln_eps;
    if (two) { e.resid_lo = ws.y_lo; e.out_lo = ws.x1_lo; e.lo8 = lo8; }
    e.reverse = OM_WALK(); e.rows_dev = k.rows_dev;
    RUN(omk_gemm(dt, ffa, F, lw.ffn2_w, F, dt, ws.x1, H, Mg, H, F, e, s));
    RUN(omk_ln_stats_reduce(ws.slots, nslots, Mg, st2, s));
  }
#undef OM_WALK
  const OmLayerWeights& last = Ls[c->n_layers - 1];
  *out = EncStream{ws.x1, two ? ws.x1_lo : nullptr, lo8, last.ln2_g, last.ln2_b, 0, ws.x};
  return 0;
}

static int bert_pending_ln(const EncCall& k, EncStream* out) {
  ENC_LOCALS;
  NOMIC_LOCALS;
  const float scale = 1.0f / sqrtf((float)c->head_dim);
  float* const y_a = ws.y32;
  float* const y_b = ws.r32b;
  for (int l = 0; l < c->n_layers; ++l) {
    const OmLayerWeights& lw = Ls[l];
    float* const st1 = ws.stats1 + (size_t)l * M * 2;
    float* const st2p = l ? ws.stats2 + (size_t)(l - 1) * M * 2 : nullptr;
    GemmEpilogue e = {};
    e.bias = lw.qkv_b; e.ln_eps = c->ln_eps;
    if (l) { e.a_ln32 = y_b; e.a_ln_g = Ls[l - 1].ln2_g; e.a_ln_b = Ls[l - 1].ln2_b; e.a_ln_stats_out = st2p; }
    RUN(omk_gemm(dt, ws.x, H, lw.qkv_w, H, dt, ws.qkv, 3 * H, Mg, 3 * H, H, e, s));
    NOMIC_ROPE();
    RUN(omk_attention(dt, ws.qkv, ws.ctx, k.mask, k.posbias, B, (int)L, H, nh, scale, 0.f, 0, s, 0, ws.kmax));
    e = GemmEpilogue{};
    e.bias = lw.o_b; e.ldr = H; e.out32 = y_a; e.ln_eps = c->ln_eps;
    if (l) { e.rln32 = y_b; e.rln32_stats = st2p; e.rln_g = Ls[l - 1].ln2_g; e.rln_b = Ls[l - 1].ln2_b; }
    else e.resid32 = ws.r32a;
    RUN(omk_gemm(dt, ws.ctx, H, lw.o_w, H, dt, ws.y, H, Mg, H, H, e, s));
    e = GemmEpilogue{};
    e.bias = lw.ffn1_b; e.act = act1; e.ln_eps = c->ln_eps;
    e.a_ln32 = y_a; e.a_ln_g = lw.ln1_g; e.a_ln_b = lw.ln1_b; e.a_ln_stats_out = st1;
    RUN(omk_gemm(dt, ws.x1, H, lw.ffn1_w, H, dt, ws.ff, F1, Mg, F1, H, e, s));
    NOMIC_SWIGLU();
    e = GemmEpilogue{};
    e.bias = lw.ffn2_b; e.ldr = H; e.out32 = y_b; e.ln_eps = c->ln_eps;
    e.rln32 = y_a; e.rln32_stats = st1; e.rln_g = lw.ln1_g; e.rln_b = lw.ln1_b;
    RUN(omk_gemm(dt, ffa, F, lw.ffn2_w, F, dt, ws.y, H, Mg, H, F, e, s));
  }
  const OmLayerWeights& last = Ls[c->n_layers - 1];
  void* dst = k.out_hidden ? k.out_hidden : (void*)ws.x;
  RUN(omk_layernorm_dual(dt, y_b, H, dst, ws.r32a, H, last.ln2_g, last.ln2_b, M, H, c->ln_eps, s));
  *out = EncStream{};
  out->hidden = (char*)dst; out->rows32 = ws.r32a;
  return 0;
}

static int bert_few32(const EncCall& k, EncStream* out) {
  ENC_LOCALS;
  NOMIC_LOCALS;
  const float scale = 1.0f / sqrtf((float)c->head_dim);
  void* dst = ws.x;
  for (int l = 0; l < c->n_layers; ++l) {
    const OmLayerWeights& lw = Ls[l];
    GEMM(ws.x, H, lw.qkv_w, H, ws.qkv, 3 * H, 3 * H, H, lw.qkv_b, nullptr, 0, OM_ACT_NONE);
    NOMIC_ROPE();
    RUN(omk_attention(dt, ws.qkv, ws.ctx, k.mask, k.posbias, B, (int)L, H, nh, scale, 0.f, 0, s, 0, ws.kmax));
    GemmEpilogue e = {};
    e.bias = lw.o_b; e.resid32 = ws.r32a; e.ldr = H; e.out32 = ws.y32;
    RUN(omk_gemm(dt, ws.ctx, H, lw.o_w, H, dt, ws.y, H, Mg, H, H, e, s));
    RUN(omk_layernorm_dual(dt, ws.y32, H, ws.x1, ws.r32b, H, lw.ln1_g, lw.ln1_b, M, H, c->ln_eps, s));
    GEMM(ws.x1, H, lw.ffn1_w, H, ws.ff, F1, F1, H, lw.ffn1_b, nullptr, 0, act1);
    NOMIC_SWIGLU();
    e = GemmEpilogue{};
    e.bias = lw.ffn2_b; e.resid32 = ws.r32b; e.ldr = H; e.out32 = ws.y32;
    RUN(omk_gemm(dt, ffa, F, lw.ffn2_w, F, dt, ws.y, H, Mg, H, F, e, s));
    if (l == c->n_layers - 1 && k.out_hidden) dst = k.out_hidden;
    RUN(omk_layernorm_dual(dt, ws.y32, H, dst, ws.r32a, H, lw.ln2_g, lw.ln2_b, M, H, c->ln_eps, s));
  }
  *out = EncStream{};
  out->hidden = (char*)dst; out->rows32 = ws.r32a;
  return 0;
}

static int bert_plain(const EncCall& k, EncStream* out) {
  ENC_LOCALS;
  NOMIC_LOCALS;
  const float scale = 1.0f / sqrtf((float)c->head_dim);
  for (int l = 0; l < c->n_layers; ++l) {
    const OmLayerWeights& lw = Ls[l];
    if (l) RUN(omk_layernorm(dt, ws.y, H, ws.x, H, Ls[l - 1].ln2_g, Ls[l - 1].ln2_b, M, H, c->ln_eps, 0, s));
    GEMM(ws.x, H, lw.qkv_w, H, ws.qkv, 3 * H, 3 * H, H, lw.qkv_b, nullptr, 0, OM_ACT_NONE);
    NOMIC_ROPE();
    RUN(omk_attention(dt, ws.qkv, ws.ctx, k.mask, k.posbias, B, (int)L, H, nh, scale, 0.f, 0, s, 0, ws.kmax));
    GEMM(ws.ctx, H, lw.o_w, H, ws.y, H, H, H, lw.o_b, ws.x, H, OM_ACT_NONE);
    RUN(omk_layernorm(dt, ws.y, H, ws.x1, H, lw.ln1_g, lw.ln1_b, M, H, c->ln_eps, 0, s));
    GEMM(ws.x1, H, lw.ffn1_w, H, ws.ff, F1, F1, H, lw.ffn1_b, nullptr, 0, act1);
    NOMIC_SWIGLU();
    GEMM(ffa, F, lw.ffn2_w, F, ws.y, H, H, F, lw.ffn2_b, ws.x1, H, OM_ACT_NONE);
  }
  *out = EncStream{};
  if (c->n_layers > 0) *out = EncStream{ws.y, nullptr, 0, Ls[c->n_layers - 1].ln2_g, Ls[c->n_layers - 1].ln2_b, 0, ws.x};
  else out->hidden = ws.x;
  return 0;
}

static int modernbert(const EncCall& k, EncStream* out) {
  ENC_LOCALS;
  const float scale = 1.0f / sqrtf((float)c->head_dim);
  for (int l = 0; l < c->n_layers; ++l) {
    const OmLayerWeights& lw = Ls[l];
    if (!lw.ffn1g_w) OM_FAIL("ModernBERT layers need the gate half of Wi (ffn1g_w)");
    const void* a_in = ws.x;
    if (lw.ln1_g) {
      RUN(omk_layernorm(dt, ws.x, H, ws.y, H, lw.ln1_g, lw.ln1_b, M, H, c->ln_eps, 0, s));
      a_in = ws.y;
    }
    GEMM(a_in, H, lw.qkv_w, H, ws.qkv, 3 * H, 3 * H, H, lw.qkv_b, nullptr, 0, OM_ACT_NONE);
    const bool sliding = ((c->sliding_layers >> l) & 1) != 0;
    RUN(omk_rope(dt, ws.qkv, M, (int)L, H, sliding ? c->rope_theta_local : c->rope_theta_global, s));
    RUN(omk_attention(dt, ws.qkv, ws.ctx, k.mask, nullptr, B, (int)L, H, nh, scale, 0.f, 0, s, 0, ws.kmax, nullptr, sliding ? c->half_window : 0));
    GEMM(ws.ctx, H, lw.o_w, H, ws.x, H, H, H, lw.o_b, ws.x, H, OM_ACT_NONE);
    RUN(omk_layernorm(dt, ws.x, H, ws.y, H, lw.ln2_g, lw.ln2_b, M, H, c->ln_eps, 0, s));
    GEMM(ws.y, H, lw.ffn1g_w, H, ws.ff2, F, F, H, nullptr, nullptr, 0, OM_ACT_NONE);
    GEMM(ws.y, H, lw.ffn1_w, H, ws.ff, F, F, H, lw.ffn1_b, ws.ff2, F, c->act | OM_ACT_MUL_RESID);
    GEMM(ws.ff, F, lw.ffn2_w, F, ws.x, H, H, F, lw.ffn2_b, ws.x, H, OM_ACT_NONE);
  }
  *out = EncStream{ws.x, nullptr, 0, k.w->final_ln_g, k.w->final_ln_b, 0, ws.y};
  return 0;
}

static int t5_fused(const EncCall& k, EncStream* out) {
  ENC_LOCALS;
  const float inv_h = 1.0f / (float)H;
  const int nslots = 2 * (H / 256);
  auto folded = [&](int layer_, bool ffn1_, const void* A_, const void* W_, const float* g_, const float* stats_, void* C_, int N_, int act_,
                    const void* res_, int64_t ldr_) -> int {
    const void* wf; const float *cs, *bfp;
    if (folded_weights(c, k.w, layer_, ffn1_, W_, g_, nullptr, nullptr, N_, H, ws.wfold, ws.colsum, ws.bfold, s, &wf, &cs, &bfp)) return 1;
    (void)cs; (void)bfp;
    GemmEpilogue e = {};
    e.act = act_; e.resid = res_; e.ldr = ldr_;
    e.ln_stats = stats_; e.ln_rms = 1; e.ln_inv_h = inv_h; e.ln_eps = c->ln_eps; e.rows_dev = k.rows_dev;
    return omk_gemm(dt, A_, H, wf, H, dt, C_, N_, Mg, N_, H, e, s);
  };
  for (int l = 0; l < c->n_layers; ++l) {
    const OmLayerWeights& lw = Ls[l];
    float* st1 = ws.stats1 + (size_t)l * Mg * 2;
    float* st2 = ws.stats2 + (size_t)l * Mg * 2;
    if (l == 0) {
      RUN(omk_layernorm(dt, ws.x, H, ws.y, H, lw.ln1_g, nullptr, M, H, c->ln_eps, 1, s));
      GemmEpilogue e0 = {};
      e0.rows_dev = k.rows_dev;
      RUN(omk_gemm(dt, ws.y, H, lw.qkv_w, H, dt, ws.qkv, 3 * H, Mg, 3 * H, H, e0, s));
    } else {
      RUN(folded(l, false, ws.x, lw.qkv_w, lw.ln1_g, ws.stats2 + (size_t)(l - 1) * Mg * 2, ws.qkv, 3 * H, OM_ACT_NONE, nullptr, 0));
    }
    RUN(omk_attention(dt, ws.qkv, ws.ctx, k.mask, k.posbias, B, (int)L, H, nh, 1.0f, 0.f, 0, s, 0, ws.kmax, k.cu));
    GemmEpilogue e = {};
    e.resid = ws.x; e.ldr = H; e.stats_out = ws.slots; e.ln_inv_h = inv_h; e.ln_eps = c->ln_eps; e.rows_dev = k.rows_dev;
    RUN(omk_gemm(dt, ws.ctx, H, lw.o_w, H, dt, ws.x, H, Mg, H, H, e, s));
    RUN(omk_ln_stats_reduce(ws.slots, nslots, Mg, st1, s));
    RUN(folded(l, true, ws.x, lw.ffn1_w, lw.ln2_g, st1, ws.ff, F, c->act, nullptr, 0));
    e = GemmEpilogue{};
    e.resid = ws.x; e.ldr = H; e.stats_out = ws.slots; e.ln_inv_h = inv_h; e.ln_eps = c->ln_eps; e.rows_dev = k.rows_dev;
    RUN(omk_gemm(dt, ws.ff, F, lw.ffn2_w, F, dt, ws.x, H, Mg, H, F, e, s));
    RUN(omk_ln_stats_reduce(ws.slots, nslots, Mg, st2, s));
  }
  *out = EncStream{ws.x, nullptr, 0, k.w->final_ln_g, nullptr, 1, ws.y};
  return 0;
}

static int t5_plain(const EncCall& k, EncStream* out) {
  ENC_LOCALS;
  for (int l = 0; l < c->n_layers; ++l) {
    const OmLayerWeights& lw = Ls[l];
    RUN(omk_layernorm(dt, ws.x, H, ws.y, H, lw.ln1_g, nullptr, M, H, c->ln_eps, 1, s));
    GEMM(ws.y, H, lw.qkv_w, H, ws.qkv, 3 * H, 3 * H, H, nullptr, nullptr, 0, OM_ACT_NONE);
    RUN(omk_attention(dt, ws.qkv, ws.ctx, k.mask, k.posbias, B, (int)L, H, nh, 1.0f, 0.f, 0, s, 0, ws.kmax));
    GEMM(ws.ctx, H, lw.o_w, H, ws.x, H, H, H, nullptr, ws.x, H, OM_ACT_NONE);
    RUN(omk_layernorm(dt, ws.x, H, ws.y, H, lw.ln2_g, nullptr, M, H, c->ln_eps, 1, s));
    if (lw.ffn1g_w) {
      GEMM(ws.y, H, lw.ffn1g_w, H, ws.ff2, F, F, H, nullptr, nullptr, 0, OM_ACT_NONE);
      GEMM(ws.y, H, lw.ffn1_w, H, ws.ff, F, F, H, nullptr, ws.ff2, F, c->act | OM_ACT_MUL_RESID);
    } else {
      GEMM(ws.y, H, lw.ffn1_w, H, ws.ff, F, F, H, nullptr, nullptr, 0, c->act);
    }
    GEMM(ws.ff, F, lw.ffn2_w, F, ws.x, H, H, F, nullptr, ws.x, H, OM_ACT_NONE);
  }
  *out = EncStream{ws.x, nullptr, 0, k.w->final_ln_g, nullptr, 1, ws.y};
  return 0;
}

static int final_norm(const EncCall& k, const EncStream& n, char** hidden, const float** rows32, int64_t* n32) {
  const OmEncoderConfig* c = k.c; const EncWs& ws = k.ws; hipStream_t s = k.s;
  const int dt = c->dtype, H = c->hidden;
  const int64_t B = k.B, L = k.L, M = k.p.M;
  const bool pooled32 = dt != OM_F32 && c->pooling != OM_POOL_NONE;
  *hidden = n.hidden; *rows32 = ws.final32; *n32 = 0;
  if (!n.x) {
    if (n.rows32 && c->pooling != OM_POOL_NONE) { *rows32 = n.rows32; *n32 = M; }
    return 0;
  }
  if (k.out_hidden || !pooled32) {
    void* dst = k.out_hidden ? k.out_hidden : n.spare;
    RUN(omk_layernorm(dt, n.x, H, dst, H, n.g, n.b, M, H, c->ln_eps, n.rms, s, n.x_lo, n.lo8));
    *hidden = (char*)dst;
  }
  if (pooled32 && c->pooling == OM_POOL_FIRST) {
    const int* rows = k.cu ? ws.cls_rows : nullptr;
    RUN(omk_layernorm_f32out(dt, n.x, rows ? H : L * H, ws.final32, H, n.g, n.b, B, H, c->ln_eps, n.rms, s, n.x_lo, rows, n.lo8));
    *n32 = B;
  } else if (pooled32) {
    RUN(omk_layernorm_f32out(dt, n.x, H, ws.final32, H, n.g, n.b, M, H, c->ln_eps, n.rms, s, n.x_lo, nullptr, n.lo8));
    *n32 = M;
  }
  return 0;
}

int omk_pooled_tail(const OmEncoderConfig* c, const OmEncoderWeights* w, const float* pooled, float* out_reps, int64_t B, const int* cu,
                    int64_t packed_rows, hipStream_t s) {
  int D = c->hidden;
  if (c->head_in > 0 && w->head_w) {
    D = c->head_out;
    RUN(om_gemm_nt(OM_F32, pooled, c->hidden, w->head_w, c->head_in, OM_F32, out_reps, D, B, D, c->head_in, nullptr, nullptr, 0, OM_ACT_NONE, s));
  }
  if (c->normalize) RUN(omk_l2norm(out_reps, out_reps, B, D, s));
  if (cu) RUN(omk_pack_overflow_poison(cu, B, packed_rows, out_reps, B * (int64_t)D, s));
  return 0;
}

static int skip_pad_buffer(hipStream_t s, size_t ints, int** out) {
  struct Buf { int* p = nullptr; size_t n = 0; bool captured = false; };
  static std::mutex mu;
  static std::map<std::pair<int, hipStream_t>, Buf> bufs;
  *out = nullptr;
  int dev = 0;
  OM_HIP(hipGetDevice(&dev));
  hipStreamCaptureStatus st = hipStreamCaptureStatusNone;
  if (hipStreamIsCapturing(s, &st) != hipSuccess) {
    (void)hipGetLastError();
    return 0;
  }
  const bool capturing = st != hipStreamCaptureStatusNone;
  std::lock_guard<std::mutex> lk(mu);
  Buf& b = bufs[std::make_pair(dev, s)];
  if (b.n < ints) {
    if (capturing) return 0;
    if (b.p && !b.captured) { OM_HIP(hipDeviceSynchronize()); OM_HIP(hipFree(b.p)); }
    b = Buf{};
    OM_HIP(hipMalloc(&b.p, ints * sizeof(int)));
    b.n = ints;
  }
  b.captured |= capturing;
  *out = b.p;
  return 0;
}

static int encoder_forward_impl(const OmEncoderConfig* c, const OmEncoderWeights* w,
                                const int64_t* input_ids, const int64_t* attention_mask,
                                const int64_t* token_type_ids, int64_t B, int64_t L,
                                void* out_hidden, float* out_reps, void* workspace,
                                size_t workspace_bytes, void* stream, int64_t packed_rows) {
  if (!c || !w || !input_ids || !attention_mask) OM_FAIL("null argument");
  if (check_cfg(c)) return 1;
  if (B <= 0) return 0;
  const OmLayerWeights* Ls = w->layers_host;
  if (!Ls) OM_FAIL("layers_host is null");
  const EncPlanIn plan_in = {c, B, L, packed_rows, out_hidden != nullptr, c->n_layers > 0 && Ls[0].ffn1g_w != nullptr, w->rel_bias != nullptr,
                             w->type_emb != nullptr};
  const EncSwitches sw = encoder_switches();
  const EncPlan plan = encoder_plan_checked(plan_in, sw);
  const bool bert = enc_bert_family(c);
  if (om_option(OM_OPT_ENCODER_DEBUG) && plan.path && bert)
    fprintf(stderr, "om_encoder_forward: M=%ld fused_ln=%d packed=%d few_rows=%d pending_ln=%d L=%ld head_dim=%d rel_bias=%d\n", (long)plan.M,
            (int)(plan.path == OM_ENC_PATH_BERT_FUSED), (int)(packed_rows > 0), (int)plan.few_rows, (int)(plan.path == OM_ENC_PATH_BERT_PENDING_LN), (long)L,
            c->head_dim, (int)plan.rel_bias);
  if (om_option(OM_OPT_ENCODER_DEBUG) && plan.path && c->arch == OM_ARCH_T5)
    fprintf(stderr, "om_encoder_forward (t5): M=%ld fused_norm=%d packed=%d\n", (long)plan.M, (int)(plan.path == OM_ENC_PATH_T5_FUSED), (int)(packed_rows > 0));
  if (plan.error) OM_FAIL(plan.error);
  if (c->arch == OM_ARCH_T5 && !w->final_ln_g) OM_FAIL("T5 needs rel_bias and final_ln_g");
  if (c->arch == OM_ARCH_MODERNBERT && (!w->emb_ln_g || !w->final_ln_g)) OM_FAIL("ModernBERT needs emb_ln_g and final_ln_g");
  if (c->arch == OM_ARCH_NOMICBERT && (!w->type_emb || w->pos_emb || w->rel_bias)) OM_FAIL("NomicBERT needs type_emb and takes no pos_emb or rel_bias");
  if (!workspace || ((uintptr_t)workspace & 255)) OM_FAIL("workspace must be 256-byte aligned");
  EncWs ws = carve(c, plan, B, L, packed_rows, (char*)workspace);
  if (ws.total > workspace_bytes) OM_FAIL("workspace too small");
  if (c->pooling != OM_POOL_NONE && !out_reps) OM_FAIL("out_reps required when pooling is set");
  hipStream_t s = (hipStream_t)stream;
  const int dt = c->dtype, H = c->hidden;
  const int64_t M = plan.M;
  int64_t pack_bound = packed_rows;
  bool skip = false;
  if (encoder_skip_pad(plan_in, plan, sw)) {
    int* side = nullptr;
    RUN(skip_pad_buffer(s, (size_t)(plan.Mp + 2 * B + 2), &side));
    if (side) {
      skip = true;
      pack_bound = plan.Mp;
      ws.cu = side; ws.cls_rows = side + (B + 2); ws.row_map = ws.cls_rows + B;
    }
  }
  const bool packed = pack_bound > 0;
  const int* const row_map = packed ? ws.row_map : nullptr;

  RUN(omk_mask_extent(attention_mask, B, (int)L, ws.kmax, s));
  if (packed) RUN(omk_pack_rows(ws.kmax, B, (int)L, pack_bound, ws.cu, ws.cls_rows, ws.row_map, s));
  if (plan.rel_bias) {
    const int* lut = nullptr;
    RUN(om_t5_lut_device((int)L, c->rel_buckets, c->rel_max_dist, &lut));
    RUN(omk_t5_bias(w->rel_bias, lut, ws.posbias, (int)L, c->n_heads, s));
  }
  const bool few32 = plan.path == OM_ENC_PATH_BERT_FEW32 || plan.path == OM_ENC_PATH_BERT_PENDING_LN;
  if (bert)
    RUN(omk_embed(dt, input_ids, token_type_ids, w->word_emb, w->pos_emb, w->type_emb, w->emb_ln_g, w->emb_ln_b, ws.x, M, (int)L, H,
                  c->vocab, c->type_vocab, c->ln_eps, 1, s, row_map, few32 ? ws.r32a : nullptr));
  else if (c->arch == OM_ARCH_MODERNBERT)
    RUN(omk_embed(dt, input_ids, nullptr, w->word_emb, nullptr, nullptr, w->emb_ln_g, w->emb_ln_b, ws.x, M, (int)L, H, c->vocab, 1, c->ln_eps, 1, s));
  else
    RUN(omk_embed(dt, input_ids, nullptr, w->word_emb, nullptr, nullptr, nullptr, nullptr, ws.x, M, (int)L, H, c->vocab, 1, c->ln_eps, 0, s, row_map));

  const EncCall k = {c, w, attention_mask, B, L, plan, ws, plan.rel_bias ? ws.posbias : nullptr, packed ? ws.cu : nullptr, row_map, out_hidden, s,
                     skip ? ws.cu + B : nullptr};
  EncStream stream_out;
  switch (plan.path) {
    case OM_ENC_PATH_BERT_FUSED: RUN(bert_fused(k, &stream_out)); break;
    case OM_ENC_PATH_BERT_PENDING_LN: RUN(bert_pending_ln(k, &stream_out)); break;
    case OM_ENC_PATH_BERT_FEW32: RUN(bert_few32(k, &stream_out)); break;
    case OM_ENC_PATH_BERT_PLAIN: RUN(bert_plain(k, &stream_out)); break;
    case OM_ENC_PATH_MODERNBERT: RUN(modernbert(k, &stream_out)); break;
    case OM_ENC_PATH_T5_FUSED: RUN(t5_fused(k, &stream_out)); break;
    case OM_ENC_PATH_T5_PLAIN: RUN(t5_plain(k, &stream_out)); break;
    default: OM_FAIL("no path planned");
  }
  char* final_hidden;
  const float* f32_rows;
  int64_t final32_rows;
  RUN(final_norm(k, stream_out, &final_hidden, &f32_rows, &final32_rows));

  if (c->pooling != OM_POOL_NONE) {
    float* pooled = c->head_in > 0 && w->head_w ? ws.pooled : out_reps;
    if (final32_rows == B && c->pooling == OM_POOL_FIRST && (f32_rows == ws.final32 || L == 1))
      OM_HIP(hipMemcpyAsync(pooled, f32_rows, (size_t)B * H * 4, hipMemcpyDeviceToDevice, s));
    else if (final32_rows == M)
      RUN(omk_pool(OM_F32, f32_rows, attention_mask, pooled, B, (int)L, H, c->pooling, s, k.cu));
    else
      RUN(omk_pool(dt, final_hidden, attention_mask, pooled, B, (int)L, H, c->pooling, s));
    RUN(omk_pooled_tail(c, w, pooled, out_reps, B, k.cu, pack_bound, s));
  }
  return 0;
}
#undef NOMIC_SWIGLU
#undef NOMIC_ROPE
#undef NOMIC_LOCALS
#undef ENC_LOCALS
#undef GEMM
#undef RUN

extern "C" int om_encoder_forward(const OmEncoderConfig* c, const OmEncoderWeights* w,
                                  const int64_t* input_ids, const int64_t* attention_mask,
                                  const int64_t* token_type_ids, int64_t B, int64_t L,
                                  void* out_hidden, float* out_reps, void* workspace,
                                  size_t workspace_bytes, void* stream) {
  return encoder_forward_impl(c, w, input_ids, attention_mask, token_type_ids, B, L, out_hidden, out_reps, workspace, workspace_bytes, stream, 0);
}

extern "C" int om_encoder_forward_packed(const OmEncoderConfig* c, const OmEncoderWeights* w,
                                         const int64_t* input_ids, const int64_t* attention_mask,
                                         const int64_t* token_type_ids, int64_t B, int64_t L, int64_t packed_rows,
                                         float* out_reps, void* workspace, size_t workspace_bytes, void* stream) {
  if (packed_rows <= 0) OM_FAIL("packed_rows must be positive");
  return encoder_forward_impl(c, w, input_ids, attention_mask, token_type_ids, B, L, nullptr, out_reps, workspace, workspace_bytes, stream, packed_rows);
}
```

openmatch_amd/csrc/encoder_plan.h:

```cpp
#pragma once
#include <algorithm>

#include "kernels.h"

bool omk_gemm_skinny_ok(int in_dtype, int out_dtype, int64_t M, int64_t N, int64_t K, const GemmEpilogue& ep, int max_m);

struct EncSwitches {
  int fused_ln;
  int two_plane;
  int pingpong;
  int skinny_m;
  int few_ln_fuse;
  int attention_fast;
  int skip_pad;
};

static EncSwitches encoder_switches() {
  return EncSwitches{om_option(OM_OPT_ENCODER_FUSED_LN), om_option(OM_OPT_ENCODER_TWO_PLANE), om_option(OM_OPT_ENCODER_PINGPONG),
                     om_option(OM_OPT_GEMM_SKINNY_M), om_option(OM_OPT_FEW_ROWS_LN_FUSE), om_option(OM_OPT_ATTENTION_FAST),
                     om_option(OM_OPT_ENCODER_SKIP_PAD)};
}

struct EncPlanIn {
  const OmEncoderConfig* c;
  int64_t B, L, packed_rows;
  bool want_hidden;
  bool gated_ffn, has_rel_bias, has_type_emb;
};

struct EncPlan {
  int path;
  const char* error;
  int64_t M;
  int64_t Mp;
  int64_t Mg;
  bool few_rows;
  bool two;
  int lo8;
  bool pingpong;
  bool rel_bias;
  bool alloc_few32;
};

static const char* encoder_cfg_error(const OmEncoderConfig* c) {
  if (c->dtype != OM_F32 && c->dtype != OM_BF16 && c->dtype != OM_F16) return "dtype must be OM_F32, OM_BF16 or OM_F16";
  if (c->dtype == OM_F16 && c->arch == OM_ARCH_BERT && c->act != OM_ACT_GELU_ERF) return "float16 mode: erf-GELU BERT-family encoders only";
  if (c->dtype == OM_F16 && c->arch == OM_ARCH_T5 && c->act != OM_ACT_RELU && c->act != OM_ACT_GELU_TANH)
    return "float16 mode: T5 feed-forwards with ReLU or tanh-GELU only";
  if (c->arch != OM_ARCH_BERT && c->arch != OM_ARCH_T5 && c->arch != OM_ARCH_MODERNBERT && c->arch != OM_ARCH_NOMICBERT) return "unknown arch";
  if (c->arch == OM_ARCH_NOMICBERT) {
    if (c->head_dim != 64 || c->n_heads * 64 != c->hidden) return "NomicBERT: only head_dim 64 with n_heads*64 == hidden is supported";
    if (c->act != OM_ACT_SILU) return "NomicBERT: hidden_act must be \"silu\"";
    if (!(c->rope_theta_global > 0.f)) return "NomicBERT: a positive rope theta";
    if (c->rel_buckets != 0) return "NomicBERT: no relative position bias (rel_buckets must be 0)";
    if (c->hidden % 64 || c->ffn % 64 || c->ffn < 64) return "NomicBERT: hidden and ffn must be multiples of 64";
  }
  if (c->arch == OM_ARCH_MODERNBERT) {
    if (c->head_dim != 64 || c->n_heads * 64 != c->hidden) return "ModernBERT: only head_dim 64 with n_heads*64 == hidden is supported";
    if (c->act != OM_ACT_GELU_ERF) return "ModernBERT: hidden_activation must be \"gelu\" (erf)";
    if (c->n_layers > 64) return "ModernBERT: at most 64 layers";
    if (!(c->rope_theta_global > 0.f) || !(c->rope_theta_local > 0.f) || c->half_window < 0)
      return "ModernBERT: positive rope thetas and a non-negative half window";
  }
  if (c->arch == OM_ARCH_T5 && (c->head_dim != 64 || c->n_heads * 64 != c->hidden))
    return "T5 encoders: only d_kv 64 with n_heads*64 == d_model is supported";
  if ((c->head_dim != 32 && c->head_dim != 64) || c->n_heads * c->head_dim != c->hidden)
    return "head_dim must be 32 or 64 with n_heads*head_dim == hidden";
  if (c->arch == OM_ARCH_BERT && c->rel_buckets != 0 && (c->rel_buckets < 4 || c->rel_buckets % 2 || c->rel_max_dist <= c->rel_buckets / 4))
    return "relative position bias: an even number of buckets >= 4 and a maximum distance beyond the exact buckets";
  const int es = c->dtype == OM_F32 ? 4 : 2;
  if ((c->hidden * es) % 128 || (c->ffn * es) % 128) return "hidden/ffn rows must be multiples of 128 bytes";
  if (c->head_in > 0 && ((c->head_in * 4) % 128 || c->head_in != c->hidden)) return "head_in must equal hidden";
  return nullptr;
}

static inline bool enc_bert_family(const OmEncoderConfig* c) { return c->arch == OM_ARCH_BERT || c->arch == OM_ARCH_NOMICBERT; }
static inline int enc_ffn1_cols(const OmEncoderConfig* c) { return c->arch == OM_ARCH_NOMICBERT ? 2 * c->ffn : c->ffn; }

static bool enc_ln_fusable(int dt, int64_t rows, int H, int F, int F1) {
  return omk_gemm_ln_fusable(dt, rows, H, H) && omk_gemm_ln_fusable(dt, rows, F1, H) && omk_gemm_ln_fusable(dt, rows, 3 * H, H) &&
         omk_gemm_ln_fusable(dt, rows, H, F);
}

static bool enc_pending_ln_ok(int dt, int64_t M, int H, int F, int F1, int act, int max_m) {
  static const float one = 1.f;
  GemmEpilogue a = {}, r = {};
  a.a_ln32 = &one; a.a_ln_g = &one; a.a_ln_b = &one;
  r.rln32 = &one; r.rln32_stats = &one; r.rln_g = &one; r.rln_b = &one; r.out32 = const_cast<float*>(&one);
  GemmEpilogue f = a;
  f.act = act;
  return omk_gemm_skinny_ok(dt, dt, M, 3 * (int64_t)H, H, a, max_m) && omk_gemm_skinny_ok(dt, dt, M, F1, H, f, max_m) &&
         omk_gemm_skinny_ok(dt, dt, M, H, H, r, max_m) && omk_gemm_skinny_ok(dt, dt, M, H, F, r, max_m);
}

static EncPlan encoder_plan_checked(const EncPlanIn& in, const EncSwitches sw) {
  const OmEncoderConfig* c = in.c;
  EncPlan p = {};
  auto run = [&](int path) { p.path = path; return p; };
  auto refuse = [&](const char* why) { p.error = why; return p; };
  const int dt = c->dtype, H = c->hidden, F = c->ffn, F1 = enc_ffn1_cols(c);
  const bool half = dt == OM_BF16 || dt == OM_F16, packed = in.packed_rows > 0, bert = enc_bert_family(c), nomic = c->arch == OM_ARCH_NOMICBERT;
  p.M = packed ? in.packed_rows : in.B * in.L;
  p.Mp = half && p.M >= 512 ? (p.M + 255) / 256 * 256 : p.M;
  p.alloc_few32 = half && bert && !packed && p.M <= (int64_t)std::max(0, sw.skinny_m);
  if (in.B <= 0) return p;
  if (in.L < 1 || in.L > 1024) return refuse("sequence length must be in [1,1024]");
  if (packed) {
    if (dt == OM_F32 || in.want_hidden || c->pooling == OM_POOL_NONE || c->n_layers < 1)
      return refuse("packed rows: 16-bit inference that returns representations only");
    if (in.packed_rows % 256 || in.packed_rows < 512 || in.packed_rows > in.B * in.L + 255)
      return refuse("packed_rows: a multiple of 256 in [512, B * L + 255]");
  }
  p.few_rows = !packed && half && p.M <= (int64_t)sw.skinny_m && !(dt == OM_BF16 && bert && p.M >= 512 && (sw.two_plane & 1) != 0);
  p.Mg = p.few_rows ? p.M : p.Mp;
  const bool fusable = sw.fused_ln != 0 && !p.few_rows && c->n_layers > 0 && H % 8 == 0 && enc_ln_fusable(dt, p.Mg, H, F, F1);
  if (c->arch == OM_ARCH_MODERNBERT) {
    if (packed) return refuse("packed rows: not for ModernBERT (om_encoder_packed_supported is 0)");
    return run(OM_ENC_PATH_MODERNBERT);
  }
  if (!bert) {
    if (!in.has_rel_bias) return refuse("T5 needs rel_bias and final_ln_g");
    p.rel_bias = true;
    p.path = fusable && !in.gated_ffn ? OM_ENC_PATH_T5_FUSED : OM_ENC_PATH_T5_PLAIN;
    if (packed && p.path != OM_ENC_PATH_T5_FUSED) return refuse("packed rows need the fused 16-bit path (T5: widths of 256, no gated feed-forward)");
    return p;
  }
  if (in.L > c->max_pos) return refuse(nomic ? "NomicBERT: sequence longer than max_pos (max_position_embeddings)" : "sequence longer than the position table");
  if (in.has_rel_bias != (c->rel_buckets > 0)) return refuse("relative position bias: rel_bias and rel_buckets must be set together");
  if (in.has_type_emb && c->type_vocab <= 0) return refuse("token types: a type_emb table needs type_vocab > 0");
  p.rel_bias = in.has_rel_bias;
  const bool plane = (sw.two_plane & (dt == OM_BF16 ? 1 : 2)) != 0;
  if (fusable && (c->act == OM_ACT_GELU_ERF || nomic)) {
    p.two = plane;
    p.lo8 = plane && dt == OM_F16 && (sw.two_plane & 4) ? 1 : 0;
    p.pingpong = sw.pingpong != 0;
    return run(OM_ENC_PATH_BERT_FUSED);
  }
  const bool few32 = p.few_rows && c->n_layers > 0 && plane;
  p.path = !few32 ? OM_ENC_PATH_BERT_PLAIN
           : p.M <= (int64_t)sw.few_ln_fuse && enc_pending_ln_ok(dt, p.Mg, H, F, F1, nomic ? OM_ACT_NONE : c->act, sw.skinny_m) ? OM_ENC_PATH_BERT_PENDING_LN
                                                                                                       : OM_ENC_PATH_BERT_FEW32;
  if (packed) return refuse("packed rows need the fused 16-bit path (hidden, ffn multiples of 256; erf-GELU)");
  return p;
}

static EncPlan encoder_plan(const EncPlanIn& in, const EncSwitches sw) {
  if (const char* why = encoder_cfg_error(in.c)) {
    EncPlan p = {};
    p.error = why;
    return p;
  }
  return encoder_plan_checked(in, sw);
}

static bool encoder_packed_ok(const OmEncoderConfig* c, bool gated_ffn, int64_t B, int64_t L, int64_t packed_rows, const EncSwitches sw) {
  if (!c || B <= 0 || packed_rows <= 0) return false;
  if ((c->dtype != OM_BF16 && c->dtype != OM_F16) || (!enc_bert_family(c) && c->arch != OM_ARCH_T5)) return false;
  if (B * L <= (int64_t)sw.skinny_m) return false;
  if (c->dtype == OM_BF16 && !sw.attention_fast) return false;
  if (c->arch == OM_ARCH_T5 && c->dtype == OM_F16 && c->act != OM_ACT_RELU) return false;
  OmEncoderConfig q = *c;
  q.pooling = OM_POOL_FIRST;
  q.max_pos = 1024;
  const bool rel = c->arch == OM_ARCH_T5 || c->rel_buckets > 0;
  const EncPlan p = encoder_plan_checked(EncPlanIn{&q, B, L, packed_rows, false, gated_ffn, rel, false}, sw);
  return p.path && !p.error;
}

static bool encoder_skip_pad(const EncPlanIn& in, const EncPlan& p, const EncSwitches sw) {
  if (!sw.skip_pad || in.packed_rows != 0 || in.want_hidden || in.c->pooling == OM_POOL_NONE) return false;
  if (p.error || (p.path != OM_ENC_PATH_BERT_FUSED && p.path != OM_ENC_PATH_T5_FUSED)) return false;
  return encoder_packed_ok(in.c, in.gated_ffn, in.B, in.L, p.Mp, sw);
}
```

openmatch_amd/csrc/kernels.h:

```cpp
#pragma once
#include "common.h"

int omk_ln_fold(int dtype , const void* W, const float* gamma, const float* beta, const float* b, void* Wf,
                float* colsum, float* bf, int N, int K, hipStream_t s);
int omk_layernorm(int dtype, const void* x, int64_t ldx, void* y, int64_t ldy, const float* g,
                  const float* b, int64_t M, int H, float eps, int rms, hipStream_t s,
                  const void* x_lo = nullptr ,
                  int lo8 = 0 );
int omk_layernorm_dual(int dtype, const float* x, int64_t ldx, void* y, float* y32, int64_t ldy, const float* g, const float* b,
                       int64_t M, int H, float eps, hipStream_t s);
int omk_layernorm_f32out(int dtype, const void* x, int64_t ldx, float* y, int64_t ldy, const float* g, const float* b,
                         int64_t M, int H, float eps, int rms, hipStream_t s, const void* x_lo = nullptr,
                         const int* rows = nullptr ,
                         int lo8 = 0 );
int omk_layernorm_from_f32(int dtype, const float* x, int64_t ldx, void* y, int64_t ldy, const float* g, const float* b, int64_t M, int H,
                           float eps, int rms, hipStream_t s);
int omk_embed(int dtype, const int64_t* ids, const int64_t* type_ids, const float* word,
              const float* pos, const float* type, const float* g, const float* b, void* out,
              int64_t M, int L, int H, int vocab, int type_vocab, float eps, int bert,
              hipStream_t s, const int* row_map = nullptr ,
              float* out32 = nullptr );
int omk_pool(int dtype, const void* x, const int64_t* mask, float* out, int64_t B, int L, int H,
             int mode, hipStream_t s, const int* cu = nullptr );
int omk_l2norm(const float* x, float* y, int64_t M, int D, hipStream_t s);
int omk_swiglu_rows(int dtype, const void* in, void* out, int64_t M, int F, hipStream_t s);
void omk_row_note(int word);
int omk_t5_bias(const float* table, const int* lut, float* out, int L, int heads, hipStream_t s);

int omk_attention(int dtype, const void* qkv, void* ctx, const int64_t* mask,
                  const float* pos_bias, int64_t B, int L, int H, int heads, float scale,
                  float drop_p, uint64_t seed, hipStream_t s, int reverse = 0 ,
                  const int* kmax = nullptr ,
                  const int* cu = nullptr ,
                  int w = 0 );
struct AttnPlan;
int omk_attention_d32(const AttnPlan& p, int dtype, const void* qkv, void* ctx, const int64_t* mask, const float* pos_bias, int64_t B, int L,
                      int H, int heads, float scale, float drop_p, uint64_t seed, hipStream_t s, int reverse, const int* kmax, const int* cu);
int omk_rope(int dtype, void* qkv, int64_t M, int L, int H, float theta, hipStream_t s,
             const int* row_map = nullptr );
int omk_attention_band(int dtype, const void* qkv, void* ctx, const int64_t* mask, int64_t B, int L, int H, int heads, float scale,
                       int w, const int* kmax, hipStream_t s);
int omk_rope_gqa(int dtype, void* qkv, int64_t M, int L, int heads, int kv_heads, const float* inv_freq_host, float scaling, hipStream_t s,
                 const int* row_map = nullptr );
int omk_attention_causal(int dtype, const void* qkv, void* ctx, const int64_t* mask, int64_t B, int L, int heads, int kv_heads, float scale,
                         const int* kmax, hipStream_t s);
int omk_attention_causal_packed(int dtype, const void* qkv, void* ctx, const int64_t* mask, int64_t B, int L, int heads, int kv_heads, float scale,
                                const int* cu, hipStream_t s);
int omk_attention_causal_d128(int dtype, const void* qkv, void* ctx, const int64_t* mask, int64_t B, int L, int heads, int kv_heads, float scale,
                              const int* kmax, hipStream_t s);
int omk_attention_causal_d128_packed(int dtype, const void* qkv, void* ctx, const int64_t* mask, int64_t B, int L, int heads, int kv_heads,
                                     float scale, const int* cu, hipStream_t s);
int omk_qknorm_rope(int dtype, void* qkv, int64_t M, int L, int heads, int kv_heads, int head_dim, const float* q_norm_g, const float* k_norm_g,
                    float eps, const float* inv_freq_host, float scaling, hipStream_t s, const int* row_map = nullptr,
                    int gemma = 0 );
int omk_attention_gqa_d256(int dtype, const void* qkv, void* ctx, const int64_t* mask, int64_t B, int L, int heads, int kv_heads, float scale, int w,
                           const int* kmax, hipStream_t s);
int omk_attention_gqa_d256_packed(int dtype, const void* qkv, void* ctx, const int64_t* mask, int64_t B, int L, int heads, int kv_heads, float scale,
                                  int w, const int* cu, hipStream_t s);
int omk_rmsnorm_add(int dtype, const void* h, int64_t ldh, float* x, int64_t ldx, const float* g, int64_t M, int H, float eps, hipStream_t s);
int omk_rope_table(const float* inv_freq, int n, float scaling, const float2** out);
int omk_causal_debug_kmax(int64_t B, int** out);
int omk_pack_rows(const int* kmax, int64_t B, int L, int64_t rows, int* cu, int* cls_rows, int* row_map, hipStream_t s);
int omk_pack_overflow_poison(const int* cu, int64_t B, int64_t rows, float* out, int64_t n, hipStream_t s);
int omk_mask_extent(const int64_t* mask, int64_t B, int L, int* kmax, hipStream_t s);
int omk_pooled_tail(const OmEncoderConfig* c, const OmEncoderWeights* w, const float* pooled, float* out_reps, int64_t B, const int* cu,
                    int64_t packed_rows, hipStream_t s);

#define OM_ACT_GELU_ERF_GRAD 4
struct GemmEpilogue {
  const float* bias;
  const void* resid;
  int64_t ldr;
  int act;
  void* pre_act;
  int64_t ldp;
  float drop_p;
  uint64_t seed;
  const int* drop_rows;
  unsigned long long* trace;
  const float* ln_stats;
  const float* ln_colsum;
  const float* rln_stats;
  const float* rln_g;
  const float* rln_b;
  float* stats_out;
  const void* resid_lo;
  void* out_lo;
  const float* resid32;
  float* out32;
  const float* a_ln32;
  const float* a_ln_g;
  const float* a_ln_b;
  float* a_ln_stats_out;
  const float* rln32;
  const float* rln32_stats;
  int lo8;
  float ln_inv_h, ln_eps;
  int ln_rms;
  int reverse;
  const int* rows_dev;
};
__host__ __device__ inline size_t omk_lo8_offset(int64_t m, int64_t n, int64_t N) {
  const int64_t tile = (m >> 8) * (N >> 8) + (n >> 8);
  const int wave = (int)(((m >> 7) & 1) * 2 + ((n >> 7) & 1));
  const int r = (int)(m & 127), c = (int)(n & 127);
  const int P = 2 * (r >> 5) + (c >> 6);
  const int G = 2 * ((r >> 4) & 1) + ((c >> 5) & 1);
  const int lane = ((c >> 2) & 3) * 16 + (r & 15);
  return ((size_t)((tile * 4 + wave) * 8 + P)) * 2048 + (size_t)((G >> 1) * 1024 + lane * 16 + (G & 1) * 8 + ((c >> 4) & 1) * 4 + (c & 3));
}
int omk_ln_stats_reduce(const float* slots, int nslots, int64_t M, float* out, hipStream_t s);
struct GemmPlan { int family; const char* error; int act ; bool resid, train ; int lnf ; };
inline int gemm_lnf(const GemmEpilogue& ep, bool f16) {
  return ep.ln_stats ? 1 : ((ep.rln_stats || ep.stats_out) ? (ep.out_lo ? (ep.lo8 && f16 ? 4 : 3) : 2) : 0);
}
inline bool gemm_whole_tiles(int64_t M, int64_t N, int64_t K) { return M % 256 == 0 && N % 256 == 0 && (K * 2) % 128 == 0; }
bool omk_gemm_ln_fusable(int dtype, int64_t M, int64_t N, int64_t K);
unsigned long long* omk_debug_trace();
bool omk_gemm_tn_ok(int dtype, int64_t M, int64_t N, int64_t K, int64_t lda, int64_t ldb);
int omk_gemm_tn(int dtype, const void* A, int64_t lda, const void* B, int64_t ldb, float* C, int64_t ldc, float* bias,
                int64_t M, int64_t N, int64_t K, hipStream_t s);
bool omk_gemm_tn_batch_ok(int dtype, int64_t M, int64_t N, int64_t K, int64_t lda, int64_t ldb);
int omk_gemm_tn_batch(int dtype, const OmTnProblem* probs, int n, int64_t M, hipStream_t s);
bool omk_gemm_wide6_b16_has(int in_dtype, int out_dtype, int act, bool train, bool resid);
int omk_gemm_wide6_b16(int in_dtype, const void* A, int64_t lda, const void* B, int64_t ldb, int out_dtype,
                       void* C, int64_t ldc, int64_t M, int64_t N, int64_t K, const GemmEpilogue& ep, hipStream_t s);
bool omk_gemm_wide6_f32_has(int in_dtype, int out_dtype, int act, bool train, bool resid);
int omk_gemm_wide6_f32(int in_dtype, const void* A, int64_t lda, const void* B, int64_t ldb, int out_dtype,
                       void* C, int64_t ldc, int64_t M, int64_t N, int64_t K, const GemmEpilogue& ep, hipStream_t s);
int omk_gemm(int in_dtype, const void* A, int64_t lda, const void* B, int64_t ldb, int out_dtype,
             void* C, int64_t ldc, int64_t M, int64_t N, int64_t K, const GemmEpilogue& ep,
             hipStream_t s);
void omk_gemm_note(int family);

int omk_gemm_splitk(int in_dtype, const void* A, int64_t lda, const void* B, int64_t ldb, float* C,
                    int64_t ldc, int64_t M, int64_t N, int64_t K, hipStream_t s);

__host__ __device__ inline uint64_t om_hash64(uint64_t seed, uint64_t idx) {
  uint64_t x = idx * 0x9E3779B97F4A7C15ull + seed;
  x ^= x >> 32; x *= 0xD6E8FEB86659FD93ull;
  x ^= x >> 32; x *= 0xD6E8FEB86659FD93ull;
  x ^= x >> 32;
  return x;
}
struct DropCfg {
  uint32_t thresh;
  float keep_scale;
  __host__ __device__ explicit DropCfg(float p) {
    thresh = p > 0.f ? (uint32_t)(p * 65536.0f + 0.5f) : 0u;
    if (thresh > 65535u) thresh = 65535u;
    keep_scale = 65536.0f / (float)(65536u - thresh);
  }
};
__host__ __device__ inline uint64_t dropout_bits(uint64_t seed, uint64_t group) { return om_hash64(seed, group); }
__host__ __device__ inline bool dropout_field(uint64_t bits, int e, uint32_t thresh) {
  return ((uint32_t)(bits >> (16 * e)) & 0xffffu) >= thresh;
}
__host__ __device__ inline bool dropout_keep(uint64_t seed, uint64_t idx, uint32_t thresh) {
  return dropout_field(dropout_bits(seed, idx >> 2), (int)(idx & 3), thresh);
}
```

openmatch_amd/native.py:

```python
import ctypes as C
import os

import torch

_HERE = os.path.dirname(os.path.abspath(__file__))
LIB_PATH = os.path.join(_HERE, "csrc", "libopenmatch_hip.so")

OM_F32, OM_BF16, OM_F16 = 0, 1, 2
ACT_NONE, ACT_GELU_ERF, ACT_RELU, ACT_GELU_TANH = 0, 1, 2, 3
ACT_SILU = 5
ACT_MUL_RESID = 0x100
ACT_GELU_ERF_GRAD, ACT_PRE_GRAD = 4, 0x200
ARCH_BERT, ARCH_T5, ARCH_MODERNBERT, ARCH_CAUSAL, ARCH_NOMICBERT, ARCH_GEMMA3 = 0, 1, 2, 3, 4, 5
POOL_NONE, POOL_FIRST, POOL_MEAN, POOL_LAST = 0, 1, 2, 3
OPT_TRAIN_WGRAD_BATCH, OPT_GEMM_MAX_GRID, OPT_GEMM_CONT = 14, 15, 16
OPT_GEMM_GROUP_M, OPT_GEMM_VARIANT, OPT_GEMM_SKINNY_M = 6, 12, 19
GEMM_FAMILY = {"v1": 1, "v2": 2, "v6": 6, "g7": 7, "g7_one_tile": 70, "7c16": 71, "7r16": 72, "skinny": 9}
ATTN_FAMILY = {"generic": 1, "fwd16": 2, "fwd16_kmax4": 3, "fwd16c": 4, "long": 5, "d32": 6, "band16": 7, "band32": 8}
ATTN_BWD_FAMILY = {"bwd16": 1, "generic": 2, "long": 3, "d32": 4}
ENC_PATH = {"bert_fused": 1, "bert_pending_ln": 2, "bert_few32": 3, "bert_plain": 4, "modernbert": 5, "t5_fused": 6, "t5_plain": 7}
OPT_ATTENTION_FAST = 2
SEARCH_F32, SEARCH_F16_RESCORE = 0, 1
ABI_VERSION = 6

# ... 10 lines not shown
    _fields_ = [("arch", c_int), ("dtype", c_int), ("hidden", c_int), ("n_layers", c_int),
                ("n_heads", c_int), ("head_dim", c_int), ("ffn", c_int), ("vocab", c_int),
                ("max_pos", c_int), ("type_vocab", c_int), ("act", c_int), ("ln_eps", c_float),
                ("rel_buckets", c_int), ("rel_max_dist", c_int), ("pooling", c_int),
                ("head_in", c_int), ("head_out", c_int), ("normalize", c_int),
                ("rope_theta_global", c_float), ("rope_theta_local", c_float), ("half_window", c_int),
                ("sliding_layers", C.c_uint64)]


class OmCausalConfig(C.Structure):
    _fields_ = [("base", OmEncoderConfig), ("n_kv_heads", c_int), ("rope_attention_scaling", c_float), ("inv_freq", c_float * 32)]


class OmCausalConfig2(C.Structure):
    _fields_ = [("base", OmCausalConfig), ("qk_norm", c_int), ("reserved", c_int), ("inv_freq", c_float * 64)]


class OmCausalQkNorm(C.Structure):
    _fields_ = [("q_norm_g", c_void_p), ("k_norm_g", c_void_p)]


class OmGemma3Config(C.Structure):
    _fields_ = [("base", OmCausalConfig), ("attn_scale", c_float), ("half_window", c_int), ("sliding_layers", C.c_uint64),
                ("full_scaling", c_float), ("sliding_scaling", c_float), ("attn_logit_softcapping", c_float), ("bidirectional", c_int),
                ("full_inv_freq", c_float * 128), ("sliding_inv_freq", c_float * 128)]


class OmGemma3Norms(C.Structure):
    _fields_ = [(n, c_void_p) for n in ("q_norm_g", "k_norm_g", "post_attention_norm_g", "post_feedforward_norm_g")]


class OmEncoderWeights(C.Structure):
    _fields_ = [("word_emb", c_void_p), ("pos_emb", c_void_p), ("type_emb", c_void_p),
                ("emb_ln_g", c_void_p), ("emb_ln_b", c_void_p),
                ("layers_host", C.POINTER(OmLayerWeights)), ("final_ln_g", c_void_p),
                ("rel_bias", c_void_p), ("head_w", c_void_p), ("folded", c_void_p), ("final_ln_b", c_void_p)]


class OmTnProblem(C.Structure):
    _fields_ = [("A", c_void_p), ("B", c_void_p), ("C", c_void_p), ("bias", c_void_p),
                ("lda", c_int64), ("ldb", c_int64), ("ldc", c_int64), ("N", c_int64), ("K", c_int64)]


class OmT5DecoderLayer(C.Structure):
    _fields_ = [(n, c_void_p) for n in (
        "sa_v_w", "sa_o_w", "sa_ln_g", "ca_q_w", "ca_kv_w", "ca_o_w", "ca_ln_g", "ffn1_w", "ffn1g_w", "ffn2_w", "ffn_ln_g")]


class OmT5DecoderWeights(C.Structure):
    _fields_ = [("start_emb", c_void_p), ("final_ln_g", c_void_p),
                ("layers_host", C.POINTER(OmT5DecoderLayer)), ("n_layers", c_int)]


class OmT5DecoderLayerGrads(C.Structure):
    _fields_ = [(n, c_void_p) for n in (
        "sa_v_w", "sa_o_w", "sa_ln_g", "ca_q_w", "ca_kv_w", "ca_o_w", "ca_ln_g", "ffn1_w", "ffn1g_w", "ffn2_w", "ffn_ln_g")]


class OmT5DecoderGrads(C.Structure):
    _fields_ = [("start_emb", c_void_p), ("final_ln_g", c_void_p), ("layers_host", C.POINTER(OmT5DecoderLayerGrads))]


class OmAdamTensor(C.Structure):
    _fields_ = [("p", c_void_p), ("g", c_void_p), ("m", c_void_p), ("v", c_void_p), ("shadow0", c_void_p), ("shadow1", c_void_p),
                ("n", c_int64), ("weight_decay", c_float), ("shadow0_dtype", c_int), ("shadow1_dtype", c_int), ("reserved", c_int)]


class OmDebugGemmEpilogue(C.Structure):
    _fields_ = [("bias", c_void_p), ("resid", c_void_p), ("ldr", c_int64), ("act", c_int),
                ("pre_act", c_void_p), ("ldp", c_int64), ("drop_p", c_float), ("seed", C.c_uint64), ("drop_rows", c_void_p),
                ("ln_stats", c_void_p), ("ln_colsum", c_void_p), ("rln_stats", c_void_p), ("rln_g", c_void_p), ("rln_b", c_void_p),
                ("stats_out", c_void_p), ("resid_lo", c_void_p), ("out_lo", c_void_p), ("resid32", c_void_p), ("out32", c_void_p),
                ("a_ln32", c_void_p), ("a_ln_g", c_void_p), ("a_ln_b", c_void_p), ("a_ln_stats_out", c_void_p), ("rln32", c_void_p),
                ("rln32_stats", c_void_p), ("lo8", c_int), ("ln_inv_h", c_float), ("ln_eps", c_float), ("ln_rms", c_int),
                ("reverse", c_int), ("rows_dev", c_void_p)]


class OmLnSite(C.Structure):
    _fields_ = [("partial", c_void_p), ("dg", c_void_p), ("db", c_void_p), ("blocks", c_int)]


ROW_KERNEL = {"fwd_generic": 1, "fwd_x8": 2, "ln_bwd": 3}
OPT_TRAIN_WGRAD_STREAM = 8
ADAM_CHUNK = 16384


class OmLayerGrads(C.Structure):
    _fields_ = [(n, c_void_p) for n in (
        "qkv_w", "qkv_b", "o_w", "o_b", "ln1_g", "ln1_b", "ffn1_w", "ffn1_b", "ffn2_w", "ffn2_b",
        "ln2_g", "ln2_b", "ffn1g_w")]


class OmEncoderGrads(C.Structure):
    _fields_ = [("word_emb", c_void_p), ("pos_emb", c_void_p), ("type_emb", c_void_p),
                ("emb_ln_g", c_void_p), ("emb_ln_b", c_void_p),
                ("layers_host", C.POINTER(OmLayerGrads)), ("head_w", c_void_p),
                ("final_ln_g", c_void_p), ("rel_bias", c_void_p)]


_SIGNATURES = {
    "om_last_error": (C.c_char_p, []),
    "om_abi_version": (c_int, []),
    "om_device_count": (c_int, []),
    "om_debug_gemm_trace": (None, [c_void_p]),
    "om_debug_gemm_gen": (None, [c_int]),
    "om_debug_option": (c_int, [c_int, c_int]),
    "om_debug_option_value": (c_int, [c_int]),
    "om_debug_gemm_last": (c_int, []),
    "om_debug_gemm_plan": (c_int, [c_int, c_void_p, c_int64, c_void_p, c_int64, c_int, c_void_p, c_int64,
                                   c_int64, c_int64, c_int64, c_void_p, c_void_p, c_int64, c_int]),
    "om_debug_gemm_ex": (c_int, [c_int, c_void_p, c_int64, c_void_p, c_int64, c_int, c_void_p, c_int64,
                                 c_int64, c_int64, c_int64, C.POINTER(OmDebugGemmEpilogue), c_void_p]),
    "om_debug_gemm_plan_ex": (c_int, [c_int, c_void_p, c_int64, c_void_p, c_int64, c_int, c_void_p, c_int64,
                                      c_int64, c_int64, c_int64, C.POINTER(OmDebugGemmEpilogue)]),
    "om_debug_gemm_splitk": (c_int, [c_int, c_void_p, c_int64, c_void_p, c_int64, c_void_p, c_int64, c_int64, c_int64, c_int64, c_void_p]),
    "om_debug_attention": (c_int, [c_void_p, c_void_p, c_void_p, c_int64, c_int, c_int, c_int, c_void_p]),
    "om_debug_attention_ex": (c_int, [c_int, c_void_p, c_void_p, c_void_p, c_void_p, c_int64, c_int, c_int, c_int, c_float, c_float,
                                      C.c_uint64, c_void_p, c_int, c_void_p, c_void_p, c_int]),
    "om_debug_rope": (c_int, [c_int, c_void_p, c_int64, c_int, c_int, c_float, c_void_p]),
    "om_debug_rope_rows": (c_int, [c_int, c_void_p, c_int64, c_int, c_int, c_float, c_void_p, c_void_p]),
    "om_debug_swiglu_rows": (c_int, [c_int, c_void_p, c_void_p, c_int64, c_int, c_void_p]),
    "om_debug_embed": (c_int, [c_int, c_void_p, c_void_p, c_void_p, c_void_p, c_void_p, c_void_p, c_void_p, c_void_p, c_int64, c_int, c_int,
                               c_int, c_int, c_float, c_void_p]),
    "om_debug_attention_causal": (c_int, [c_int, c_void_p, c_void_p, c_void_p, c_int64, c_int, c_int, c_int, c_float, c_void_p]),
    "om_debug_rope_gqa": (c_int, [c_int, c_void_p, c_int64, c_int, c_int, c_int, C.POINTER(c_float), c_float, c_void_p]),
    "om_debug_attention_causal_packed": (c_int, [c_int, c_void_p, c_void_p, c_void_p, c_void_p, c_int64, c_int, c_int, c_int, c_float, c_void_p]),
    "om_debug_rope_gqa_rows": (c_int, [c_int, c_void_p, c_int64, c_int, c_int, c_int, C.POINTER(c_float), c_float, c_void_p, c_void_p]),
    "om_debug_attention_causal_hd": (c_int, [c_int, c_void_p, c_void_p, c_void_p, c_int64, c_int, c_int, c_int, c_int, c_float, c_void_p]),
    "om_debug_attention_causal_hd_packed": (c_int, [c_int, c_void_p, c_void_p, c_void_p, c_void_p, c_int64, c_int, c_int, c_int, c_int, c_float,
                                                    c_void_p]),
    "om_debug_qknorm_rope": (c_int, [c_int, c_void_p, c_int64, c_int, c_int, c_int, c_int, c_void_p, c_void_p, c_float, C.POINTER(c_float),
                                     c_float, c_void_p]),
    "om_debug_qknorm_rope_rows": (c_int, [c_int, c_void_p, c_int64, c_int, c_int, c_int, c_int, c_void_p, c_void_p, c_float, C.POINTER(c_float),
                                          c_float, c_void_p, c_void_p]),
    "om_debug_attention_gqa_d256": (c_int, [c_int, c_void_p, c_void_p, c_void_p, c_int64, c_int, c_int, c_int, c_float, c_int, c_void_p]),
    "om_debug_qknorm_rope_d256": (c_int, [c_int, c_void_p, c_int64, c_int, c_int, c_int, c_void_p, c_void_p, c_float, C.POINTER(c_float), c_float,
                                          c_void_p]),
    "om_debug_attention_gqa_d256_packed": (c_int, [c_int, c_void_p, c_void_p, c_void_p, c_void_p, c_int64, c_int, c_int, c_int, c_float, c_int,
                                                   c_void_p]),
    "om_debug_qknorm_rope_d256_rows": (c_int, [c_int, c_void_p, c_int64, c_int, c_int, c_int, c_void_p, c_void_p, c_float, C.POINTER(c_float),
                                               c_float, c_void_p, c_void_p]),
    "om_debug_rmsnorm_add": (c_int, [c_int, c_void_p, c_int64, c_void_p, c_int64, c_void_p, c_int64, c_int, c_float, c_void_p]),
    "om_debug_mask_extent": (c_int, [c_void_p, c_int64, c_int, c_void_p, c_void_p]),
    "om_debug_pack_rows": (c_int, [c_void_p, c_int64, c_int, c_int64, c_void_p, c_void_p, c_void_p, c_void_p]),
    "om_debug_attention_last": (c_int, []),
    "om_debug_attention_plan": (c_int, [c_int, c_int64, c_int, c_int, c_int, c_int, c_float, c_int, c_int, c_int]),
    "om_debug_attention_bwd_last": (c_int, []),
    "om_debug_attention_bwd_plan": (c_int, [c_int, c_int64, c_int, c_int, c_int, c_int, c_int, c_int, c_int]),
    "om_debug_attention_bwd_ex": (c_int, [c_int, c_void_p, c_void_p, c_void_p, c_void_p, c_void_p, c_void_p, c_void_p, c_void_p, c_int64, c_int,
                                          c_int, c_int, c_float, c_float, C.c_uint64, c_void_p, c_int, c_void_p]),
    "om_debug_attention_bwd_stats_bytes": (c_size_t, [c_int64, c_int]),
    "om_debug_encoder_plan": (c_int, [C.POINTER(OmEncoderConfig), c_int, c_int, c_int64, c_int64, c_int64, c_int]),
    "om_debug_encoder_skip_pad": (c_int, [C.POINTER(OmEncoderConfig), c_int, c_int, c_int64, c_int64, c_int]),
    "om_debug_attn_drop_keep": (c_int, [C.c_uint64, c_int64, c_int, c_int, c_int, c_int, c_int, c_float]),
    "om_debug_wave_sum_check": (c_int, [c_void_p, c_void_p, c_void_p, c_int64, c_void_p]),
    "om_debug_row_kernel_last": (c_int, []),
    "om_debug_layernorm": (c_int, [c_int, c_void_p, c_int64, c_void_p, c_int64, c_void_p, c_void_p, c_int64, c_int, c_float, c_int, c_void_p,
                                   c_int, c_void_p]),
    "om_debug_layernorm_f32out": (c_int, [c_int, c_void_p, c_int64, c_void_p, c_int64, c_void_p, c_void_p, c_int64, c_int, c_float, c_int,
                                          c_void_p, c_void_p, c_int, c_void_p]),
    "om_debug_layernorm_from_f32": (c_int, [c_int, c_void_p, c_int64, c_void_p, c_int64, c_void_p, c_void_p, c_int64, c_int, c_float, c_int,
                                            c_void_p]),
    "om_debug_layernorm_dual": (c_int, [c_int, c_void_p, c_int64, c_void_p, c_void_p, c_int64, c_void_p, c_void_p, c_int64, c_int, c_float,
                                        c_void_p]),
    "om_debug_norm_bwd": (c_int, [c_int, c_void_p, c_void_p, c_void_p, c_void_p, c_void_p, c_void_p, c_int64, c_int, c_float, c_int, c_void_p,
                                  c_void_p]),
    "om_debug_ln_bwd_drop": (c_int, [c_int, c_void_p, c_void_p, c_void_p, c_void_p, c_void_p, c_float, C.c_uint64, c_void_p, c_void_p, c_int64,
                                     c_int, c_float, c_void_p, c_void_p, c_void_p, C.POINTER(c_int), c_void_p, c_void_p]),
    "om_debug_ln_param_reduce": (c_int, [C.POINTER(OmLnSite), c_int, c_int, c_void_p]),
    "om_debug_embed_bwd": (c_int, [c_int, c_void_p, c_void_p, c_void_p, c_void_p, c_void_p, c_void_p, c_void_p, c_void_p, c_void_p, c_void_p,
                                   c_void_p, c_void_p, c_int64, c_int, c_int, c_int, c_int, c_float, c_void_p, c_void_p]),
    "om_debug_pool": (c_int, [c_int, c_void_p, c_void_p, c_void_p, c_int64, c_int, c_int, c_int, c_void_p, c_void_p]),
    "om_debug_pool_bwd": (c_int, [c_int, c_void_p, c_void_p, c_void_p, c_int64, c_int, c_int, c_int, c_void_p, c_void_p]),
    "om_debug_l2norm": (c_int, [c_void_p, c_void_p, c_int64, c_int, c_void_p]),
    "om_debug_l2norm_bwd": (c_int, [c_void_p, c_void_p, c_void_p, c_int64, c_int, c_void_p]),
    "om_debug_colsum": (c_int, [c_int, c_void_p, c_int64, c_int64, c_int, c_void_p, c_void_p]),
    "om_debug_dropout": (c_int, [c_int, c_void_p, c_void_p, c_int64, c_float, C.c_uint64, c_void_p, c_int, c_void_p]),
    "om_debug_ln_fold": (c_int, [c_int, c_void_p, c_void_p, c_void_p, c_void_p, c_void_p, c_void_p, c_void_p, c_int, c_int, c_void_p]),
    "om_debug_ln_stats_reduce": (c_int, [c_void_p, c_int, c_int64, c_void_p, c_void_p]),
    "om_encoder_fold_bytes": (c_size_t, [C.POINTER(OmEncoderConfig)]),
    "om_encoder_fold_weights": (c_int, [C.POINTER(OmEncoderConfig), C.POINTER(OmEncoderWeights), c_void_p, c_size_t, c_void_p]),
    "om_kernel_timing_enable": (c_int, [c_int]),
    "om_kernel_timing_read": (c_int, [c_int, C.POINTER(C.c_double), C.POINTER(c_int64), C.POINTER(C.c_double)]),
    "om_gemm_nt": (c_int, [c_int, c_void_p, c_int64, c_void_p, c_int64, c_int, c_void_p, c_int64,
                           c_int64, c_int64, c_int64, c_void_p, c_void_p, c_int64, c_int, c_void_p]),
    "om_gemm_tn_acc": (c_int, [c_int, c_void_p, c_int64, c_void_p, c_int64, c_void_p, c_int64, c_void_p,
                               c_int64, c_int64, c_int64, c_void_p]),
    "om_gemm_tn_acc_batch": (c_int, [c_int, C.POINTER(OmTnProblem), c_int, c_int64, c_void_p]),
    "om_encoder_workspace_bytes": (c_size_t, [C.POINTER(OmEncoderConfig), c_int64, c_int64]),
    "om_t5_decoder_workspace_bytes": (c_size_t, [C.POINTER(OmEncoderConfig), c_int64, c_int64]),
    "om_t5_decoder_step": (c_int, [C.POINTER(OmEncoderConfig), C.POINTER(OmT5DecoderWeights), c_void_p, c_void_p,
                                   c_int64, c_int64, c_void_p, c_void_p, c_size_t, c_void_p]),
    "om_t5_relative_bucket": (c_int, [c_int, c_int, c_int]),
    "om_encoder_forward": (c_int, [C.POINTER(OmEncoderConfig), C.POINTER(OmEncoderWeights), c_void_p,
                                   c_void_p, c_void_p, c_int64, c_int64, c_void_p, c_void_p,
                                   c_void_p, c_size_t, c_void_p]),
    "om_causal_encoder_workspace_bytes": (c_size_t, [C.POINTER(OmCausalConfig), c_int64, c_int64]),
    "om_causal_encoder_forward": (c_int, [C.POINTER(OmCausalConfig), C.POINTER(OmEncoderWeights), c_void_p, c_void_p, c_int64, c_int64,
                                          c_void_p, c_void_p, c_void_p, c_size_t, c_void_p]),
    "om_causal_encoder_packed_supported": (c_int, [C.POINTER(OmCausalConfig), c_int64, c_int64, c_int64]),
    "om_causal_encoder_workspace_bytes_packed": (c_size_t, [C.POINTER(OmCausalConfig), c_int64, c_int64, c_int64]),
    "om_causal_encoder_forward_packed": (c_int, [C.POINTER(OmCausalConfig), C.POINTER(OmEncoderWeights), c_void_p, c_void_p, c_int64, c_int64,
                                                 c_int64, c_void_p, c_void_p, c_size_t, c_void_p]),
    "om_causal2_encoder_workspace_bytes": (c_size_t, [C.POINTER(OmCausalConfig2), c_int64, c_int64]),
    "om_causal2_encoder_forward": (c_int, [C.POINTER(OmCausalConfig2), C.POINTER(OmEncoderWeights), C.POINTER(OmCausalQkNorm), c_void_p, c_void_p,
                                           c_int64, c_int64, c_void_p, c_void_p, c_void_p, c_size_t, c_void_p]),
    "om_causal2_encoder_packed_supported": (c_int, [C.POINTER(OmCausalConfig2), c_int64, c_int64, c_int64]),
    "om_causal2_encoder_workspace_bytes_packed": (c_size_t, [C.POINTER(OmCausalConfig2), c_int64, c_int64, c_int64]),
    "om_causal2_encoder_forward_packed": (c_int, [C.POINTER(OmCausalConfig2), C.POINTER(OmEncoderWeights), C.POINTER(OmCausalQkNorm), c_void_p,
                                                  c_void_p, c_int64, c_int64, c_int64, c_void_p, c_void_p, c_size_t, c_void_p]),
    "om_gemma3_encoder_workspace_bytes": (c_size_t, [C.POINTER(OmGemma3Config), c_int64, c_int64]),
    "om_gemma3_encoder_forward": (c_int, [C.POINTER(OmGemma3Config), C.POINTER(OmEncoderWeights), C.POINTER(OmGemma3Norms), c_void_p, c_void_p,
                                          c_int64, c_int64, c_void_p, c_void_p, c_void_p, c_size_t, c_void_p]),
    "om_gemma3_encoder_packed_supported": (c_int, [C.POINTER(OmGemma3Config), c_int64, c_int64, c_int64]),
    "om_gemma3_encoder_workspace_bytes_packed": (c_size_t, [C.POINTER(OmGemma3Config), c_int64, c_int64, c_int64]),
    "om_gemma3_encoder_forward_packed": (c_int, [C.POINTER(OmGemma3Config), C.POINTER(OmEncoderWeights), C.POINTER(OmGemma3Norms), c_void_p,
                                                 c_void_p, c_int64, c_int64, c_int64, c_void_p, c_void_p, c_size_t, c_void_p]),
    "om_encoder_packed_supported": (c_int, [C.POINTER(OmEncoderConfig), c_int, c_int64, c_int64, c_int64]),
    "om_encoder_workspace_bytes_packed": (c_size_t, [C.POINTER(OmEncoderConfig), c_int64, c_int64, c_int64]),
    "om_encoder_forward_packed": (c_int, [C.POINTER(OmEncoderConfig), C.POINTER(OmEncoderWeights), c_void_p,
                                          c_void_p, c_void_p, c_int64, c_int64, c_int64, c_void_p,
                                          c_void_p, c_size_t, c_void_p]),
    "om_encoder_tape_bytes": (c_size_t, [C.POINTER(OmEncoderConfig), c_int64, c_int64]),
    "om_encoder_train_workspace_bytes": (c_size_t, [C.POINTER(OmEncoderConfig), c_int64, c_int64]),
    "om_encoder_train_forward": (c_int, [C.POINTER(OmEncoderConfig), C.POINTER(OmEncoderWeights), c_void_p,
                                         c_void_p, c_void_p, c_int64, c_int64, c_float, c_float, C.c_uint64,
                                         c_void_p, c_size_t, c_void_p, c_void_p, c_size_t, c_void_p]),
    "om_encoder_train_backward": (c_int, [C.POINTER(OmEncoderConfig), C.POINTER(OmEncoderWeights), c_void_p,
                                          c_void_p, c_void_p, c_int64, c_int64, c_float, c_float, C.c_uint64,
                                          c_void_p, c_void_p, C.POINTER(OmEncoderGrads), c_void_p, c_size_t,
                                          c_void_p]),
    "om_encoder_train_packed_supported": (c_int, [C.POINTER(OmEncoderConfig), c_int64, c_int64, c_int64]),
    "om_encoder_tape_bytes_packed": (c_size_t, [C.POINTER(OmEncoderConfig), c_int64, c_int64, c_int64]),
    "om_encoder_train_workspace_bytes_packed": (c_size_t, [C.POINTER(OmEncoderConfig), c_int64, c_int64, c_int64]),
    "om_encoder_train_forward_packed": (c_int, [C.POINTER(OmEncoderConfig), C.POINTER(OmEncoderWeights), c_void_p,
                                                c_void_p, c_void_p, c_int64, c_int64, c_int64, c_float, c_float, C.c_uint64,
                                                c_void_p, c_size_t, c_void_p, c_void_p, c_size_t, c_void_p]),
    "om_encoder_train_backward_packed": (c_int, [C.POINTER(OmEncoderConfig), C.POINTER(OmEncoderWeights), c_void_p,
                                                 c_void_p, c_void_p, c_int64, c_int64, c_int64, c_float, c_float, C.c_uint64,
                                                 c_void_p, c_void_p, C.POINTER(OmEncoderGrads), c_void_p, c_size_t,
                                                 c_void_p]),
    "om_encoder_train_forward_hidden": (c_int, [C.POINTER(OmEncoderConfig), C.POINTER(OmEncoderWeights), c_void_p,
                                                c_void_p, c_void_p, c_int64, c_int64, c_float, c_float, C.c_uint64,
                                                c_void_p, c_size_t, c_void_p, c_void_p, c_size_t, c_void_p]),
    "om_encoder_train_backward_hidden": (c_int, [C.POINTER(OmEncoderConfig), C.POINTER(OmEncoderWeights), c_void_p,
                                                 c_void_p, c_void_p, c_int64, c_int64, c_float, c_float, C.c_uint64,
                                                 c_void_p, c_void_p, C.POINTER(OmEncoderGrads), c_void_p, c_size_t,
                                                 c_void_p]),
    "om_t5_decoder_tape_bytes": (c_size_t, [C.POINTER(OmEncoderConfig), c_int, c_int64, c_int64]),
    "om_t5_decoder_train_workspace_bytes": (c_size_t, [C.POINTER(OmEncoderConfig), c_int, c_int64, c_int64]),
    "om_t5_decoder_train_forward": (c_int, [C.POINTER(OmEncoderConfig), C.POINTER(OmT5DecoderWeights), c_void_p, c_void_p,
                                            c_int64, c_int64, c_float, C.c_uint64, c_void_p, c_size_t, c_void_p,
                                            c_void_p, c_size_t, c_void_p]),
    "om_t5_decoder_train_backward": (c_int, [C.POINTER(OmEncoderConfig), C.POINTER(OmT5DecoderWeights), c_void_p, c_void_p,
                                             c_int64, c_int64, c_float, C.c_uint64, c_void_p, c_void_p,
                                             C.POINTER(OmT5DecoderGrads), c_void_p, c_void_p, c_size_t, c_void_p]),
    "om_linear_f32_backward": (c_int, [c_void_p, c_void_p, c_void_p, c_void_p, c_void_p, c_int, c_int, c_int, c_void_p]),
    "om_index_to_f16": (c_int, [c_void_p, c_int64, c_int, c_void_p, c_void_p, c_void_p]),
    "om_sim_topk_workspace_bytes": (c_size_t, [c_int64, c_int, c_int]),
    "om_sim_topk": (c_int, [c_int, c_void_p, c_int64, c_void_p, c_void_p, c_void_p, c_int64, c_int,
                            c_int, c_int64, c_void_p, c_void_p, c_void_p, c_size_t, c_void_p]),
    "om_sim_topk_info": (None, [C.POINTER(c_int64)]),
    "om_topk_merge": (c_int, [c_void_p, c_void_p, c_int, c_int64, c_int, c_int, c_void_p, c_void_p,
                              c_void_p]),
    "om_contrastive_fwd_bwd": (c_int, [c_void_p, c_void_p, c_int, c_int, c_int, c_int, c_float,
                                       c_int, c_int, c_int, c_int, c_void_p, c_void_p, c_void_p,
                                       c_void_p, c_void_p, c_void_p]),
    "om_encoder_train_set_layer_events": (c_int, [c_void_p, c_int]),
    "om_comm_unique_id": (c_int, [c_void_p]),
    "om_comm_init": (c_int, [c_void_p, c_int, c_int, C.POINTER(c_void_p)]),
    "om_comm_destroy": (c_int, [c_void_p]),
    "om_comm_count": (c_int, [c_void_p, C.POINTER(c_int)]),
    "om_allgather_rows": (c_int, [c_void_p, c_void_p, c_void_p, c_int64, c_int64, c_void_p]),
    "om_allreduce_grads": (c_int, [c_void_p, c_void_p, c_int64, c_int, c_void_p]),
    "om_exchange_topk": (c_int, [c_void_p, c_int, c_void_p, c_void_p, c_int64, c_int, c_void_p, c_void_p, c_void_p]),
    "om_grad_sqnorm": (c_int, [c_void_p, c_void_p, c_int, c_void_p, c_void_p, c_void_p]),
    "om_adamw_step": (c_int, [c_void_p, c_void_p, c_int, c_float, c_float, c_float, c_float, c_int64, c_void_p, c_float, c_float,
                              c_int, c_void_p, c_void_p]),
    "om_loss_scale_update": (c_int, [c_void_p, c_void_p, c_int, c_void_p]),
    "om_contrastive_fwd_bwd_ex": (c_int, [c_void_p, c_void_p, c_int, c_int, c_int, c_void_p, c_int, c_int, c_void_p,
                                          c_float, c_int, c_int, c_int, c_int, c_void_p, c_void_p, c_void_p,
                                          c_void_p, c_void_p, c_void_p]),
}

_lib = None


class NativeError(RuntimeError):
    pass


def lib():
    global _lib
    if _lib is None:
        if not os.path.exists(LIB_PATH):
            raise NativeError(
                f"{LIB_PATH} is missing: build the HIP library first "
                "(python -m openmatch_amd._build, or __graft_entry__.build()). "
                "openmatch_amd has no CPU / eager fallback.")
        handle = C.CDLL(LIB_PATH)
        for name, (res, args) in _SIGNATURES.items():
            try:
                fn = getattr(handle, name)
            except AttributeError as e:
                raise NativeError(f"{LIB_PATH} does not export {name}; rebuild it") from e
            fn.restype, fn.argtypes = res, args
# ... 48 lines not shown
```

Baseline: 68040 passages/s.

## Run last encoder layer's post-attention work only on [CLS] rows

For first-token pooling without hidden output, the last layer gathers each sequence's [CLS] row (context, residual, LN stats) into compact buffers carved from the qkv area. The output projection, FFN GEMMs and LN-stats reduction then run on about B rows instead of all tokens, and the final layernorm reads the compact rows. The packed-row map kernel is also spread over many blocks using a binary search on prefix sums instead of one serial block. The risks are the extra gather launch and reuse of the qkv workspace as scratch, which is checked against its size.

New measurement: 71750 passages/s (median of 6 runs). +5.5%, better.

```diff
diff --git a/include/openmatch_hip.h b/include/openmatch_hip.h
--- a/include/openmatch_hip.h
+++ b/include/openmatch_hip.h
@@ -98,7 +98,8 @@
 #define OM_OPT_GEMM_SKINNY_CFG 20
 #define OM_OPT_FEW_ROWS_LN_FUSE 21
 #define OM_OPT_ENCODER_SKIP_PAD 22
-#define OM_OPT_COUNT 23
+#define OM_OPT_ENCODER_CLS_TAIL 23
+#define OM_OPT_COUNT 24
 int om_debug_option(int opt, int value);
 int om_debug_option_value(int opt);
 int om_debug_attention(const void* qkv, void* ctx, const int64_t* mask, int64_t B, int L, int H, int heads, void* stream);
@@ -167,6 +168,10 @@
 int om_debug_encoder_plan(const struct OmEncoderConfig* cfg, int gated_ffn, int has_rel_bias, int64_t B, int64_t L, int64_t packed_rows,
                           int want_hidden);
 int om_debug_encoder_skip_pad(const struct OmEncoderConfig* cfg, int gated_ffn, int has_rel_bias, int64_t B, int64_t L, int want_hidden);
+int om_debug_encoder_cls_tail(const struct OmEncoderConfig* cfg, int gated_ffn, int has_rel_bias, int64_t B, int64_t L, int64_t packed_rows,
+                              int want_hidden);
+int om_debug_gather_rows(const void* src0, void* dst0, const void* src1, void* dst1, const void* src2, void* dst2, const float* stats_src,
+                         float* stats_dst, const int* rows, int64_t B, int64_t L, int64_t Mc, int H, void* stream);
 int om_debug_attn_drop_keep(uint64_t seed, int64_t b, int h, int heads, int Lm, int q, int key, float p);
 int om_debug_wave_sum_check(const float* in, float* out_shuffle, float* out_dpp, int64_t groups, void* stream);
 #define OM_ROW_FWD_GENERIC 1
diff --git a/openmatch_amd/csrc/abi.cpp b/openmatch_amd/csrc/abi.cpp
--- a/openmatch_amd/csrc/abi.cpp
+++ b/openmatch_amd/csrc/abi.cpp
@@ -114,6 +114,8 @@
   g_opt[OM_OPT_FEW_ROWS_LN_FUSE] = e ? atoi(e) : 64;
   e = getenv("OM_ENCODER_SKIP_PAD");
   g_opt[OM_OPT_ENCODER_SKIP_PAD] = e ? atoi(e) : 1;
+  e = getenv("OM_ENCODER_CLS_TAIL");
+  g_opt[OM_OPT_ENCODER_CLS_TAIL] = e ? atoi(e) : 1;
   g_opt_init.store(true);
 }
 }
diff --git a/openmatch_amd/csrc/attention.hip b/openmatch_amd/csrc/attention.hip
--- a/openmatch_amd/csrc/attention.hip
+++ b/openmatch_amd/csrc/attention.hip
@@ -438,23 +438,36 @@
     part[tid] += v;
     __syncthreads();
   }
-  int run = part[tid] - sum;
+  const int total = part[1023];
   const int cap = (int)rows;
-  for (int64_t i = lo; i < hi; ++i) {
-    cu[i] = run < cap ? run : cap;
-    cls_rows[i] = run < cap ? run : cap - 1;
-    const int n = kmax[i];
-    for (int k = 0; k < n; ++k) if (run + k < cap) row_map[run + k] = (int)(i * L + k);
-    run += n;
-  }
-  const int total = part[1023];
-  if (tid == 1023) { cu[B] = total < cap ? total : cap; cu[B + 1] = total; }
-  for (int64_t t = total + tid; t < rows; t += 1024) row_map[t] = -1;
+  if (blockIdx.x == 0) {
+    int run = part[tid] - sum;
+    for (int64_t i = lo; i < hi; ++i) {
+      cu[i] = run < cap ? run : cap;
+      cls_rows[i] = run < cap ? run : cap - 1;
+      run += kmax[i];
+    }
+    if (tid == 1023) { cu[B] = total < cap ? total : cap; cu[B + 1] = total; }
+  }
+  for (int64_t t = (int64_t)blockIdx.x * 1024 + tid; t < rows; t += (int64_t)gridDim.x * 1024) {
+    int v = -1;
+    if (t < total) {
+      int a = 0, b = 1023;
+      while (a < b) { const int m = (a + b) >> 1; if (part[m] > (int)t) b = m; else a = m + 1; }
+      int64_t i = a * per;
+      int run = a ? part[a - 1] : 0;
+      for (int n = kmax[i]; run + n <= (int)t; n = kmax[++i]) run += n;
+      v = (int)(i * L + ((int)t - run));
+    }
+    row_map[t] = v;
+  }
 }
 int omk_pack_rows(const int* kmax, int64_t B, int L, int64_t rows, int* cu, int* cls_rows, int* row_map, hipStream_t s) {
   if (B <= 0) return 0;
   if (rows > 0x7fffffff || B * (int64_t)L > 0x7fffffff) OM_FAIL("packed rows: token counts below 2^31");
-  hipLaunchKernelGGL(pack_rows_kernel, dim3(1), dim3(1024), 0, s, kmax, B, L, rows, cu, cls_rows, row_map);
+  const int64_t slices = (rows + 1023) / 1024;
+  hipLaunchKernelGGL(pack_rows_kernel, dim3((unsigned)(slices < 1 ? 1 : slices > 1024 ? 1024 : slices)), dim3(1024), 0, s, kmax, B, L, rows, cu, cls_rows,
+                     row_map);
   OM_LAUNCH_CHECK();
   return 0;
 }
diff --git a/openmatch_amd/csrc/elementwise.hip b/openmatch_amd/csrc/elementwise.hip
--- a/openmatch_amd/csrc/elementwise.hip
+++ b/openmatch_amd/csrc/elementwise.hip
@@ -354,6 +354,49 @@
   return 0;
 }
 
+struct GatherArgs { const uint4* src[3]; uint4* dst[3]; const float2* st_src; float2* st_dst; };
+__global__ __launch_bounds__(256) void gather_rows_kernel(GatherArgs a, const int* __restrict__ rows, int64_t B, int64_t L, int64_t Mc, int vec) {
+  const int rpb = blockDim.x / vec;
+  const int64_t r = (int64_t)blockIdx.x * rpb + threadIdx.x / vec;
+  const int v = threadIdx.x % vec;
+  if (r >= Mc) return;
+  const int64_t b = r < B ? r : B - 1;
+  const int64_t sr = rows ? (int64_t)rows[b] : b * L;
+#pragma unroll
+  for (int p = 0; p < 3; ++p)
+    if (a.src[p]) a.dst[p][r * vec + v] = a.src[p][sr * vec + v];
+  if (v == 0 && a.st_src) a.st_dst[r] = a.st_src[sr];
+}
+int omk_gather_rows(const GatherPlane (&planes)[3], const float* stats_src, float* stats_dst, const int* rows, int64_t B, int64_t L, int64_t Mc,
+                    int H, hipStream_t s) {
+  if (B <= 0 || Mc <= 0) return 0;
+  if (H < 8 || H % 8 || L < 1) OM_FAIL("row gather: rows of whole 16-byte vectors");
+  GatherArgs a = {};
+  uintptr_t align = (uintptr_t)stats_src | (uintptr_t)stats_dst;
+  for (int p = 0; p < 3; ++p) {
+    if (!planes[p].src || !planes[p].dst) continue;
+    a.src[p] = (const uint4*)planes[p].src; a.dst[p] = (uint4*)planes[p].dst;
+    align |= (uintptr_t)planes[p].src | (uintptr_t)planes[p].dst;
+  }
+  if (stats_src && stats_dst) { a.st_src = (const float2*)stats_src; a.st_dst = (float2*)stats_dst; }
+  if (align & 15) OM_FAIL("row gather: 16-byte aligned buffers");
+  const int vec = H / 8;
+  const int threads = vec >= 256 ? vec : 256 / vec * vec;
+  if (threads > 256) OM_FAIL("row gather: at most 2048 columns");
+  const int64_t grid = (Mc + threads / vec - 1) / (threads / vec);
+  if (grid > 0x7fffffffLL) OM_FAIL("row gather: too many rows for one launch");
+  hipLaunchKernelGGL(gather_rows_kernel, dim3((unsigned)grid), dim3(threads), 0, s, a, rows, B, L, Mc, vec);
+  OM_LAUNCH_CHECK();
+  return 0;
+}
+extern "C" int om_debug_gather_rows(const void* src0, void* dst0, const void* src1, void* dst1, const void* src2, void* dst2, const float* stats_src,
+                                    float* stats_dst, const int* rows, int64_t B, int64_t L, int64_t Mc, int H, void* stream) {
+  if (!src0 || !dst0) OM_FAIL("om_debug_gather_rows: null argument");
+  if (B < 1 || Mc < B) OM_FAIL("om_debug_gather_rows: 1 <= B <= Mc");
+  const GatherPlane planes[3] = {{src0, dst0}, {src1, dst1}, {src2, dst2}};
+  return omk_gather_rows(planes, stats_src, stats_dst, rows, B, L, Mc, H, (hipStream_t)stream);
+}
+
 int omk_layernorm_from_f32(int dtype, const float* x, int64_t ldx, void* y, int64_t ldy, const float* g, const float* b, int64_t M, int H,
                            float eps, int rms, hipStream_t s) {
   if (H % 4 != 0 || H > 64 * 4 * MAX_VEC_LIMIT) OM_FAIL("hidden size must be a multiple of 4 and <= 2048");
diff --git a/openmatch_amd/csrc/encoder.hip b/openmatch_amd/csrc/encoder.hip
--- a/openmatch_amd/csrc/encoder.hip
+++ b/openmatch_amd/csrc/encoder.hip
@@ -179,6 +179,17 @@
   return encoder_skip_pad(in, encoder_plan(in, sw), sw) ? 1 : 0;
 }
 
+extern "C" int om_debug_encoder_cls_tail(const OmEncoderConfig* c, int gated_ffn, int has_rel_bias, int64_t B, int64_t L, int64_t packed_rows,
+                                         int want_hidden) {
+  if (!c) {
+    om_set_error("om_debug_encoder_cls_tail: null argument");
+    return -1;
+  }
+  const EncPlanIn in = {c, B, L, packed_rows, want_hidden != 0, gated_ffn != 0, has_rel_bias != 0, c->type_vocab > 0};
+  const EncSwitches sw = encoder_switches();
+  return encoder_cls_tail(in, encoder_plan(in, sw), sw) ? 1 : 0;
+}
+
 extern "C" int om_t5_relative_bucket(int relative_position, int num_buckets, int max_distance) {
   int nb = num_buckets / 2;
   int bucket = relative_position > 0 ? nb : 0;
@@ -209,6 +220,7 @@
   void* out_hidden;
   hipStream_t s;
   const int* rows_dev;
+  int64_t cls_mc;
 };
 
 struct EncStream {
@@ -220,6 +232,7 @@
   void* spare;
   char* hidden;
   const float* rows32;
+  bool cls_compact;
 };
 
 #define GEMM(A_, lda_, W_, ldw_, C_, ldc_, N_, K_, bias_, res_, ldr_, act_)                        \
@@ -237,7 +250,7 @@
   const int F1 = enc_ffn1_cols(c), act1 = nomic ? OM_ACT_NONE : c->act;                                             \
   const void* const ffa = nomic ? ws.ff2 : ws.ff
 #define NOMIC_ROPE() do { if (nomic) RUN(omk_rope(dt, ws.qkv, M, (int)L, H, c->rope_theta_global, s, k.row_map)); } while (0)
-#define NOMIC_SWIGLU() do { if (nomic) RUN(omk_swiglu_rows(dt, ws.ff, ws.ff2, Mg, F, s)); } while (0)
+#define NOMIC_SWIGLU(rows_) do { if (nomic) RUN(omk_swiglu_rows(dt, ws.ff, ws.ff2, rows_, F, s)); } while (0)
 
 static int bert_fused(const EncCall& k, EncStream* out) {
   ENC_LOCALS;
@@ -249,12 +262,24 @@
   const int nslots = 2 * (H / 256);
   const bool pingpong = k.p.pingpong;
   int walk = 1;
+  const int64_t Mc = k.cls_mc;
+  const size_t cplane = (size_t)Mc * H * 2;
+  char* const cbase = ws.qkv;
+  float* const cst2p = (float*)(cbase + 7 * cplane);
+  float* const cst1 = cst2p + 2 * Mc;
+  if (Mc > 0 && ((char*)(cst1 + 2 * Mc) > ws.qkv + (size_t)Mg * 3 * H * 2 || Mc > Mg || c->n_layers < 2 || lo8))
+    OM_FAIL("[CLS] tail: the compact buffers do not fit the qkv area");
 #define OM_WALK() (pingpong ? (walk ^= 1, walk ^ 1) : 0)
   for (int l = 0; l < c->n_layers; ++l) {
     const OmLayerWeights& lw = Ls[l];
-    float* st1 = ws.stats1 + (size_t)l * Mg * 2;
+    const bool last = l == c->n_layers - 1, tail = last && Mc > 0;
+    float* st1 = tail ? cst1 : ws.stats1 + (size_t)l * Mg * 2;
     float* st2 = ws.stats2 + (size_t)l * Mg * 2;
     const float* st2p = l ? ws.stats2 + (size_t)(l - 1) * Mg * 2 : nullptr;
+    const int64_t Mr = tail ? Mc : Mg;
+    const int* const rdev = tail ? nullptr : k.rows_dev;
+    const char *ctx = ws.ctx, *xin = ws.x1, *xin_lo = ws.x1_lo;
+    char *y = ws.y, *y_lo = ws.y_lo, *xout = ws.x1, *xout_lo = ws.x1_lo;
     GemmEpilogue e = {};
     if (l == 0) {
       e.bias = lw.qkv_b; e.reverse = OM_WALK(); e.rows_dev = k.rows_dev;
@@ -268,37 +293,44 @@
     }
     NOMIC_ROPE();
     RUN(omk_attention(dt, ws.qkv, ws.ctx, k.mask, k.posbias, B, (int)L, H, nh, scale, 0.f, 0, s, OM_WALK(), ws.kmax, k.cu));
+    if (tail) {
+      const GatherPlane planes[3] = {{ws.ctx, cbase}, {ws.x1, cbase + cplane}, {two ? ws.x1_lo : nullptr, cbase + 2 * cplane}};
+      RUN(omk_gather_rows(planes, st2p, cst2p, k.cu ? ws.cls_rows : nullptr, B, L, Mc, H, s));
+      ctx = cbase; xin = cbase + cplane; xin_lo = cbase + 2 * cplane; st2p = cst2p;
+      y = cbase + 3 * cplane; y_lo = cbase + 4 * cplane; xout = cbase + 5 * cplane; xout_lo = cbase + 6 * cplane;
+    }
     e = GemmEpilogue{};
     e.bias = lw.o_b; e.ldr = H; e.stats_out = ws.slots; e.ln_inv_h = inv_h; e.ln_eps = c->ln_eps;
-    if (two) { e.out_lo = ws.y_lo; e.lo8 = lo8; }
+    if (two) { e.out_lo = y_lo; e.lo8 = lo8; }
     if (l == 0) {
       e.resid = ws.x;
     } else {
       const OmLayerWeights& pw = Ls[l - 1];
-      e.resid = ws.x1; e.rln_stats = st2p; e.rln_g = pw.ln2_g; e.rln_b = pw.ln2_b;
-      if (two) e.resid_lo = ws.x1_lo;
-    }
-    e.reverse = OM_WALK(); e.rows_dev = k.rows_dev;
-    RUN(omk_gemm(dt, ws.ctx, H, lw.o_w, H, dt, ws.y, H, Mg, H, H, e, s));
-    RUN(omk_ln_stats_reduce(ws.slots, nslots, Mg, st1, s));
+      e.resid = xin; e.rln_stats = st2p; e.rln_g = pw.ln2_g; e.rln_b = pw.ln2_b;
+      if (two) e.resid_lo = xin_lo;
+    }
+    e.reverse = OM_WALK(); e.rows_dev = rdev;
+    RUN(omk_gemm(dt, ctx, H, lw.o_w, H, dt, y, H, Mr, H, H, e, s));
+    RUN(omk_ln_stats_reduce(ws.slots, nslots, Mr, st1, s));
     const void* wf1; const float *cs1, *bf1;
     RUN(folded_weights(c, k.w, l, true, lw.ffn1_w, lw.ln1_g, lw.ln1_b, lw.ffn1_b, F1, H, ws.wfold, ws.colsum, ws.bfold, s, &wf1, &cs1, &bf1));
     e = GemmEpilogue{};
     e.bias = bf1; e.act = act1; e.ln_stats = st1; e.ln_colsum = cs1; e.ln_inv_h = inv_h; e.ln_eps = c->ln_eps;
-    e.reverse = OM_WALK(); e.rows_dev = k.rows_dev;
-    RUN(omk_gemm(dt, ws.y, H, wf1, H, dt, ws.ff, F1, Mg, F1, H, e, s));
-    NOMIC_SWIGLU();
-    e = GemmEpilogue{};
-    e.bias = lw.ffn2_b; e.resid = ws.y; e.ldr = H; e.rln_stats = st1; e.rln_g = lw.ln1_g; e.rln_b = lw.ln1_b;
+    e.reverse = OM_WALK(); e.rows_dev = rdev;
+    RUN(omk_gemm(dt, y, H, wf1, H, dt, ws.ff, F1, Mr, F1, H, e, s));
+    NOMIC_SWIGLU(Mr);
+    e = GemmEpilogue{};
+    e.bias = lw.ffn2_b; e.resid = y; e.ldr = H; e.rln_stats = st1; e.rln_g = lw.ln1_g; e.rln_b = lw.ln1_b;
     e.stats_out = ws.slots; e.ln_inv_h = inv_h; e.ln_eps = c->ln_eps;
-    if (two) { e.resid_lo = ws.y_lo; e.out_lo = ws.x1_lo; e.lo8 = lo8; }
-    e.reverse = OM_WALK(); e.rows_dev = k.rows_dev;
-    RUN(omk_gemm(dt, ffa, F, lw.ffn2_w, F, dt, ws.x1, H, Mg, H, F, e, s));
-    RUN(omk_ln_stats_reduce(ws.slots, nslots, Mg, st2, s));
+    if (two) { e.resid_lo = y_lo; e.out_lo = xout_lo; e.lo8 = lo8; }
+    e.reverse = OM_WALK(); e.rows_dev = rdev;
+    RUN(omk_gemm(dt, ffa, F, lw.ffn2_w, F, dt, xout, H, Mr, H, F, e, s));
+    if (!last) RUN(omk_ln_stats_reduce(ws.slots, nslots, Mg, st2, s));
   }
 #undef OM_WALK
-  const OmLayerWeights& last = Ls[c->n_layers - 1];
-  *out = EncStream{ws.x1, two ? ws.x1_lo : nullptr, lo8, last.ln2_g, last.ln2_b, 0, ws.x};
+  const OmLayerWeights& lastw = Ls[c->n_layers - 1];
+  *out = EncStream{ws.x1, two ? ws.x1_lo : nullptr, lo8, lastw.ln2_g, lastw.ln2_b, 0, ws.x};
+  if (Mc > 0) { out->x = cbase + 5 * cplane; out->x_lo = two ? cbase + 6 * cplane : nullptr; out->cls_compact = true; }
   return 0;
 }
 
@@ -327,7 +359,7 @@
     e.bias = lw.ffn1_b; e.act = act1; e.ln_eps = c->ln_eps;
     e.a_ln32 = y_a; e.a_ln_g = lw.ln1_g; e.a_ln_b = lw.ln1_b; e.a_ln_stats_out = st1;
     RUN(omk_gemm(dt, ws.x1, H, lw.ffn1_w, H, dt, ws.ff, F1, Mg, F1, H, e, s));
-    NOMIC_SWIGLU();
+    NOMIC_SWIGLU(Mg);
     e = GemmEpilogue{};
     e.bias = lw.ffn2_b; e.ldr = H; e.out32 = y_b; e.ln_eps = c->ln_eps;
     e.rln32 = y_a; e.rln32_stats = st1; e.rln_g = lw.ln1_g; e.rln_b = lw.ln1_b;
@@ -356,7 +388,7 @@
     RUN(omk_gemm(dt, ws.ctx, H, lw.o_w, H, dt, ws.y, H, Mg, H, H, e, s));
     RUN(omk_layernorm_dual(dt, ws.y32, H, ws.x1, ws.r32b, H, lw.ln1_g, lw.ln1_b, M, H, c->ln_eps, s));
     GEMM(ws.x1, H, lw.ffn1_w, H, ws.ff, F1, F1, H, lw.ffn1_b, nullptr, 0, act1);
-    NOMIC_SWIGLU();
+    NOMIC_SWIGLU(Mg);
     e = GemmEpilogue{};
     e.bias = lw.ffn2_b; e.resid32 = ws.r32b; e.ldr = H; e.out32 = ws.y32;
     RUN(omk_gemm(dt, ffa, F, lw.ffn2_w, F, dt, ws.y, H, Mg, H, F, e, s));
@@ -381,7 +413,7 @@
     GEMM(ws.ctx, H, lw.o_w, H, ws.y, H, H, H, lw.o_b, ws.x, H, OM_ACT_NONE);
     RUN(omk_layernorm(dt, ws.y, H, ws.x1, H, lw.ln1_g, lw.ln1_b, M, H, c->ln_eps, 0, s));
     GEMM(ws.x1, H, lw.ffn1_w, H, ws.ff, F1, F1, H, lw.ffn1_b, nullptr, 0, act1);
-    NOMIC_SWIGLU();
+    NOMIC_SWIGLU(Mg);
     GEMM(ffa, F, lw.ffn2_w, F, ws.y, H, H, F, lw.ffn2_b, ws.x1, H, OM_ACT_NONE);
   }
   *out = EncStream{};
@@ -493,8 +525,8 @@
     *hidden = (char*)dst;
   }
   if (pooled32 && c->pooling == OM_POOL_FIRST) {
-    const int* rows = k.cu ? ws.cls_rows : nullptr;
-    RUN(omk_layernorm_f32out(dt, n.x, rows ? H : L * H, ws.final32, H, n.g, n.b, B, H, c->ln_eps, n.rms, s, n.x_lo, rows, n.lo8));
+    const int* rows = k.cu && !n.cls_compact ? ws.cls_rows : nullptr;
+    RUN(omk_layernorm_f32out(dt, n.x, rows || n.cls_compact ? H : L * H, ws.final32, H, n.g, n.b, B, H, c->ln_eps, n.rms, s, n.x_lo, rows, n.lo8));
     *n32 = B;
   } else if (pooled32) {
     RUN(omk_layernorm_f32out(dt, n.x, H, ws.final32, H, n.g, n.b, M, H, c->ln_eps, n.rms, s, n.x_lo, nullptr, n.lo8));
@@ -586,6 +618,8 @@
     }
   }
   const bool packed = pack_bound > 0;
+  int64_t cls_mc = 0;
+  if (!encoder_cls_tail(plan_in, plan, sw, &cls_mc)) cls_mc = 0;
   const int* const row_map = packed ? ws.row_map : nullptr;
 
   RUN(omk_mask_extent(attention_mask, B, (int)L, ws.kmax, s));
@@ -605,8 +639,8 @@
     RUN(omk_embed(dt, input_ids, nullptr, w->word_emb, nullptr, nullptr, nullptr, nullptr, ws.x, M, (int)L, H, c->vocab, 1, c->ln_eps, 0, s, row_map));
 
   const EncCall k = {c, w, attention_mask, B, L, plan, ws, plan.rel_bias ? ws.posbias : nullptr, packed ? ws.cu : nullptr, row_map, out_hidden, s,
-                     skip ? ws.cu + B : nullptr};
-  EncStream stream_out;
+                     skip ? ws.cu + B : nullptr, cls_mc};
+  EncStream stream_out = {};
   switch (plan.path) {
     case OM_ENC_PATH_BERT_FUSED: RUN(bert_fused(k, &stream_out)); break;
     case OM_ENC_PATH_BERT_PENDING_LN: RUN(bert_pending_ln(k, &stream_out)); break;
diff --git a/openmatch_amd/csrc/encoder_plan.h b/openmatch_amd/csrc/encoder_plan.h
--- a/openmatch_amd/csrc/encoder_plan.h
+++ b/openmatch_amd/csrc/encoder_plan.h
@@ -13,12 +13,13 @@
   int few_ln_fuse;
   int attention_fast;
   int skip_pad;
+  int cls_tail;
 };
 
 static EncSwitches encoder_switches() {
   return EncSwitches{om_option(OM_OPT_ENCODER_FUSED_LN), om_option(OM_OPT_ENCODER_TWO_PLANE), om_option(OM_OPT_ENCODER_PINGPONG),
                      om_option(OM_OPT_GEMM_SKINNY_M), om_option(OM_OPT_FEW_ROWS_LN_FUSE), om_option(OM_OPT_ATTENTION_FAST),
-                     om_option(OM_OPT_ENCODER_SKIP_PAD)};
+                     om_option(OM_OPT_ENCODER_SKIP_PAD), om_option(OM_OPT_ENCODER_CLS_TAIL)};
 }
 
 struct EncPlanIn {
@@ -172,3 +173,12 @@
   if (p.error || (p.path != OM_ENC_PATH_BERT_FUSED && p.path != OM_ENC_PATH_T5_FUSED)) return false;
   return encoder_packed_ok(in.c, in.gated_ffn, in.B, in.L, p.Mp, sw);
 }
+
+static bool encoder_cls_tail(const EncPlanIn& in, const EncPlan& p, const EncSwitches sw, int64_t* Mc = nullptr) {
+  if (!sw.cls_tail || p.error || p.path != OM_ENC_PATH_BERT_FUSED || p.lo8) return false;
+  if (in.c->pooling != OM_POOL_FIRST || in.want_hidden || in.c->n_layers < 2 || in.B < 512) return false;
+  const int64_t mc = (in.B + 255) / 256 * 256;
+  if (4 * mc > p.Mp) return false;
+  if (Mc) *Mc = mc;
+  return true;
+}
diff --git a/openmatch_amd/csrc/kernels.h b/openmatch_amd/csrc/kernels.h
--- a/openmatch_amd/csrc/kernels.h
+++ b/openmatch_amd/csrc/kernels.h
@@ -110,6 +110,9 @@
   return ((size_t)((tile * 4 + wave) * 8 + P)) * 2048 + (size_t)((G >> 1) * 1024 + lane * 16 + (G & 1) * 8 + ((c >> 4) & 1) * 4 + (c & 3));
 }
 int omk_ln_stats_reduce(const float* slots, int nslots, int64_t M, float* out, hipStream_t s);
+struct GatherPlane { const void* src; void* dst; };
+int omk_gather_rows(const GatherPlane (&planes)[3], const float* stats_src, float* stats_dst, const int* rows, int64_t B, int64_t L, int64_t Mc,
+                    int H, hipStream_t s);
 struct GemmPlan { int family; const char* error; int act ; bool resid, train ; int lnf ; };
 inline int gemm_lnf(const GemmEpilogue& ep, bool f16) {
   return ep.ln_stats ? 1 : ((ep.rln_stats || ep.stats_out) ? (ep.out_lo ? (ep.lo8 && f16 ? 4 : 3) : 2) : 0);
diff --git a/openmatch_amd/native.py b/openmatch_amd/native.py
--- a/openmatch_amd/native.py
+++ b/openmatch_amd/native.py
@@ -186,6 +186,9 @@
     "om_debug_attention_bwd_stats_bytes": (c_size_t, [c_int64, c_int]),
     "om_debug_encoder_plan": (c_int, [C.POINTER(OmEncoderConfig), c_int, c_int, c_int64, c_int64, c_int64, c_int]),
     "om_debug_encoder_skip_pad": (c_int, [C.POINTER(OmEncoderConfig), c_int, c_int, c_int64, c_int64, c_int]),
+    "om_debug_encoder_cls_tail": (c_int, [C.POINTER(OmEncoderConfig), c_int, c_int, c_int64, c_int64, c_int64, c_int]),
+    "om_debug_gather_rows": (c_int, [c_void_p, c_void_p, c_void_p, c_void_p, c_void_p, c_void_p, c_void_p, c_void_p, c_void_p, c_int64, c_int64,
+                                     c_int64, c_int, c_void_p]),
     "om_debug_attn_drop_keep": (c_int, [C.c_uint64, c_int64, c_int, c_int, c_int, c_int, c_int, c_float]),
     "om_debug_wave_sum_check": (c_int, [c_void_p, c_void_p, c_void_p, c_int64, c_void_p]),
     "om_debug_row_kernel_last": (c_int, []),
```
